# dmitrykoval/vinum

Measured on AMD Instinct MI355X. Metric: rows/sec + achieved HBM GB/s, filter->group-by over 10^9-row Arrow batches, higher is better.
Workload: dtype f64/int64; 1 GPU; configs[2]: SELECT k,sum(v),avg(v) WHERE v>63.9921875 GROUP BY k; N=1e+09 rows/GPU, G=1e+08 int64 keys, s=0.5; rows_per_gpu=1000000000, groups=100000000, group_count_hint=none: the operator samples the keys (what the reference boundary allows), parallelism=batch-sharded x1

## Files before the change

vinum_amd/csrc/vnm_agg.hip:

```cpp
#include <memory>
#include <algorithm>
#include <cmath>
#include <cstdlib>
#include <vector>

#include "vnm_agg.hpp"

namespace vnm {

constexpr uint64_t EMPTY = ~0ULL;
constexpr uint64_t LOCKED = ~0ULL - 1;
constexpr int AGG_BLOCK = 1024;
#ifndef VNM_AGG_R
#define VNM_AGG_R 8
#endif
constexpr int AGG_ROWS_PER_THREAD = VNM_AGG_R;
constexpr int AGG_TILE = AGG_BLOCK * AGG_ROWS_PER_THREAD;
constexpr int AGG_LDS_BUDGET = 128 * 1024;
constexpr int AGG_MAX_PROBES = 48;
constexpr int OG_BLOCK = 256;

struct GTable {
    uint64_t* tag;
    uint64_t* keyw;
// ... 197 lines not shown
            continue;
        }
        if (t == EMPTY) {
            uint64_t expected = EMPTY;
            if (__hip_atomic_compare_exchange_strong(&g.tag[h], &expected, LOCKED, __ATOMIC_RELAXED, __ATOMIC_RELAXED,
                                                     __HIP_MEMORY_SCOPE_AGENT)) {
                for (int i = 0; i < g.kwt; i++) st_agent(&g.keyw[(uint64_t)i * g.stride + h], kw[i]);
                asm volatile("s_waitcnt vmcnt(0)" ::: "memory");
                st_agent(&g.tag[h], tagv);
                atomicAdd(newc, 1u);
                return h;
            }
            continue;
        }
        if (t == LOCKED) continue;
        h = (h + 1) & mask;
    }
}

__device__ __forceinline__ void fold_new(const GTable& g, unsigned* s_new) {
    unsigned v = atomicExch(s_new, 0u);
    if (v) atomicAdd(&g.ctl[2], (unsigned long long)v);
}

__device__ __forceinline__ bool op_value(const AccOp& op, const vnm_dcol* cols, int64_t row, uint64_t* out) {
    if (op.kind == A_COUNT_ROWS) { *out = 1; return true; }
    const vnm_dcol& c = cols[op.col];
    if (!col_valid(c, row)) return false;
    switch (op.kind) {
        case A_COUNT_VALID: *out = 1; return true;
        case A_SUM_F64: *out = (uint64_t)__double_as_longlong(col_f64(c, row)); return true;
        case A_SUM_I64: *out = (uint64_t)col_i64(c, row); return true;
        case A_SUM_LO32: *out = (uint64_t)col_i64(c, row) & 0xFFFFFFFFULL; return true;
        case A_SUM_HI32S: *out = (uint64_t)(col_i64(c, row) >> 32); return true;
        case A_SUM_HI32U: *out = (uint64_t)col_i64(c, row) >> 32; return true;
        default:
            if (type_is_float(c.type)) *out = enc_f64(col_f64(c, row));
            else if (type_is_unsigned(c.type)) *out = (uint64_t)col_i64(c, row);
            else *out = enc_i64(col_i64(c, row));
            return true;
    }
}

__device__ __forceinline__ bool table_has_room(const AggArgs& a, unsigned* s_new) {
    fold_new(a.g, s_new);
    unsigned long long fill = __hip_atomic_load(&a.g.ctl[2], __ATOMIC_RELAXED, __HIP_MEMORY_SCOPE_AGENT);
    if ((int64_t)fill + a.margin > a.fill_limit) {
        __hip_atomic_store(&a.g.ctl[1], 1ULL, __ATOMIC_RELAXED, __HIP_MEMORY_SCOPE_AGENT);
        return false;
    }
    return true;
}

#include "vnm_agg_scan.inc"

#include "vnm_agg_tuple.inc"

#include "vnm_agg_onegroup.inc"

#include "vnm_agg_table.inc"

#include "vnm_agg_part.inc"

#include "vnm_agg_pack.inc"

#include "vnm_agg_dense.inc"

#include "vnm_agg_finalize.inc"

}

using namespace vnm;

struct DensePending {
    DFinalArgs df;
    int tb = 0, levels = 0, p1 = 0, fsplits = 1;
    int64_t nfinal = 0;
    int64_t dstride = 0;
    int64_t rows = 0;
    bool x_known = true;
    uint32_t x_inv = 0, x_exp = 0;
    bool exact_ok() const { return x_known && exact_adds_proved(((unsigned long long)x_exp << 32) | x_inv, rows); }
    std::vector<DSet> sets;
    std::vector<void*> blocks;
    DSet* dsets = nullptr;
    DTabSlot* table = nullptr;
    ~DensePending() { for (void* b : blocks) pool_free(b); pool_free(table); pool_free(dsets); }
};
constexpr size_t DP_MAX_SETS = 512;
struct DScanPending {
    DFinalArgs df{};
    DScanTable t{};
    int slots = 0;
    uint64_t* part_sum = nullptr;
    float* part_lo = nullptr;
    uint32_t* part_cnt = nullptr;
    unsigned long long* flags = nullptr;
    ~DScanPending() { pool_free(t.sum); pool_free(t.lo); pool_free(t.cnt); pool_free(part_sum); pool_free(part_lo); pool_free(part_cnt); pool_free(flags); }
};

struct vnm_agg {
    AggPlan plan;
    FuncOut outs[AGG_MAX_FUNCS];
    int n_funcs = 0;
    int func_col[AGG_MAX_FUNCS];
    int col_first_func[AGG_MAX_COLS];
    bool single = false;
    Predicate pred{};
    bool pred_set = false;
    int pred_op = 0, pred_is_float = 0;
    double pred_dval = 0;
    int64_t pred_ival = 0;
    int64_t hint = 0;
    GTable g{};
    bool have_table = false;
    int64_t rows_seen = 0;
    uint64_t* dkey = nullptr;
    uint64_t* dacc = nullptr;
    int64_t dstride = 0;
    int64_t n_groups = -1;
    std::vector<uint64_t> h_key, h_acc;
    bool host_ready = false;
    uint64_t* run_key = nullptr;
    uint64_t* run_acc = nullptr;
    int64_t run_stride = 0, run_n = 0;
    bool have_run = false;
    bool result_is_run = false;
    bool estimated = false;
    int64_t merge_stride = 0;
    unsigned long long* run_dir = nullptr;
    int64_t run_nfin = 0;
    vnm_agg* inner = nullptr;
    bool pack_tried = false;
    bool key_only_failed = false;
    int dense_state = 0;
    DenseMap dmap{};
    int64_t dense_span = 0;
    uint64_t dense_rlo = 0, dense_rhi = 0;
    bool rank_aligned = false;
    struct DensePending* pending = nullptr;
    double heavy_share = 0.0;
    int key_out_type = -1;
    std::vector<std::pair<int64_t, void*>> widened;
    bool widen_in[AGG_MAX_FUNCS] = {};
    bool any_widen_in = false;
    bool pred_lit_rounded = false;
    int pred_user_is_float = 0;
    double pred_user_dval = 0.0;
    int64_t pred_user_ival = 0;
    int fx_state = 0, fx_qe = 0;
    bool pack_null_seen = false;
    bool pring_off = false;
    bool fx_narrow = false;
    int fxn_state = 0, fxn_qe[3] = {0, 0, 0};
    bool null_inputs_seen = false;
    bool count8_off = false;
    int count_cb = 0;
    struct DScanPending* scan_pending = nullptr;
    bool dense_by_bound = false;
    bool range_given = false;
    int expr_col = -1;
    std::vector<vnm_expr_ins> expr_prog;
    int expr_ncols = 0;
    bool expr_fusable = false;
    bool expr_active = false;
    ExprProg expr_dev{};
    PackParams pack{};
    int c_funcs[AGG_MAX_FUNCS], c_in_types[AGG_MAX_FUNCS], c_in_flags[AGG_MAX_FUNCS], c_in_col_ids[AGG_MAX_FUNCS];
    bool c_has_ids = false;
    TDict tdict{};
    int64_t widest_est = 0;
    unsigned long long* tnext = nullptr;
    bool tuple_mode = false;
    std::vector<vnm_agg*> parts;
    std::vector<std::vector<int>> part_funcs;
    bool split_tried = false;
    bool async = false;
    struct QBatch { int64_t nrows; vnm_dcol key, col, pred; std::vector<vnm_dcol> ins; int64_t seq; };
    bool q_multi = false;
    std::vector<QBatch> q;
    int64_t q_rows = 0;
    bool q_pred_is_v = false;
    const std::vector<QBatch>* segs_active = nullptr;
    const uint8_t* kn_valid = nullptr;
    int64_t kn_off = 0;
    bool kn_failed = false;
    std::vector<VSeg> seg_host;
    struct vnm_agg_exact* ex = nullptr;
    bool child = false;
    int64_t seq = 0;
    int64_t cur_seq = -1;
};

namespace {

int table_alloc(vnm_agg* h, GTable* g, uint64_t cap, hipStream_t s) {
    memset(g, 0, sizeof(*g));
    g->cap = cap;
    g->stride = cap + 2;
    g->kwt = h->single || h->plan.n_keys == 0 ? 0 : h->plan.n_keys + 1;
    g->n_words = h->plan.n_words;
    g->tag = (uint64_t*)pool_alloc(g->stride * 8);
    g->acc = (uint64_t*)pool_alloc(g->stride * 8 * (size_t)g->n_words);
    g->ctl = (unsigned long long*)pool_alloc(64);
    if (g->kwt) g->keyw = (uint64_t*)pool_alloc(g->stride * 8 * (size_t)g->kwt);
    if (!g->tag || !g->acc || !g->ctl || (g->kwt && !g->keyw)) return 1;
    VNM_HIP(hipMemsetAsync(g->tag, 0xFF, g->stride * 8, s));
    VNM_HIP(hipMemsetAsync(g->ctl, 0, 64, s));
    for (int w = 0; w < g->n_words; w++) {
        const uint64_t init = merge_init(h->plan.merge[w]);
        if (init == 0 || init == ~0ULL) VNM_HIP(hipMemsetAsync(g->acc + (size_t)w * g->stride, init ? 0xFF : 0, g->stride * 8, s));
        else {
            fill_u64_kernel<<<(int)std::min<uint64_t>((g->stride + 255) / 256, (uint64_t)device_info().num_cus * 8), 256, 0, s>>>(g->acc + (size_t)w * g->stride, init, (int64_t)g->stride);
            VNM_HIP(hipGetLastError());
        }
    }
    return 0;
}

void table_free(GTable* g) {
    pool_free(g->tag);
    pool_free(g->acc);
    pool_free(g->keyw);
    pool_free(g->ctl);
    memset(g, 0, sizeof(*g));
}

uint64_t pow2_at_least(uint64_t x) {
    uint64_t p = 1;
    while (p < x) p <<= 1;
    return p;
}

int lds_slots_for(const AggPlan& p, int budget = AGG_LDS_BUDGET) {
    int per_slot = 8 * (1 + p.n_words);
    int s = 1;
    while ((s * 2 + 2) * per_slot <= budget) s *= 2;
    if (s > 8192) s = 8192;
    return s;
}

int table_grow(vnm_agg* h, uint64_t new_cap, hipStream_t s) {
    GTable old = h->g, ng;
    VNM_TRY(table_alloc(h, &ng, new_cap, s));
    MergeArgs m{};
    m.plan = h->plan;
    m.g = ng;
    m.n = (int64_t)old.stride;
    m.src_is_table = 1;
    m.src_stride = 1;
    m.src_tag = old.tag;
    m.src_cap = (int64_t)old.cap;
    for (int j = 0; j < old.kwt; j++) m.src_key[j] = old.keyw + (size_t)j * old.stride;
    for (int w = 0; w < old.n_words; w++) m.src_acc[w] = old.acc + (size_t)w * old.stride;
    int grid = device_info().num_cus * 8;
    agg_merge_kernel<<<grid, 256, 0, s>>>(m);
    VNM_HIP(hipGetLastError());
    VNM_HIP(hipStreamSynchronize(s));
    table_free(&old);
    h->g = ng;
    return 0;
}

int ensure_table(vnm_agg* h, int64_t nrows, hipStream_t s, bool rows_only = false) {
    if (h->have_table) return 0;
    uint64_t cap;
    if (h->plan.n_keys == 0) cap = 2;
    else {
        uint64_t want = h->hint > 0 ? (uint64_t)h->hint * 2 : (uint64_t)1 << 22;
        if ((h->hint <= 0 || rows_only) && (uint64_t)nrows * 2 < want) want = (uint64_t)(nrows > 512 ? nrows : 512) * 2;
        if (rows_only && want > (1ULL << 20)) want = 1ULL << 20;
        cap = pow2_at_least(want < 1024 ? 1024 : want);
    }
    VNM_TRY(table_alloc(h, &h->g, cap, s));
    h->have_table = true;
    return 0;
}

void invalidate_result(vnm_agg* h) {
    if (!h->result_is_run) {
        pool_free(h->dkey);
        pool_free(h->dacc);
    }
    h->result_is_run = false;
    h->dkey = h->dacc = nullptr;
    h->n_groups = -1;
    h->host_ready = false;
}

int64_t env_i64(const char* name, int64_t dflt) {
    const char* v = getenv(name);
    return v ? (int64_t)atoll(v) : dflt;
}

void drop_run(vnm_agg* h) {
    pool_free(h->run_key);
    pool_free(h->run_acc);
    pool_free(h->run_dir);
    h->run_dir = nullptr;
    h->run_nfin = 0;
    h->run_key = h->run_acc = nullptr;
    h->have_run = false;
    h->run_n = h->run_stride = 0;
}

int estimate_groups(vnm_agg* h, const vnm_dcol& key, int64_t nrows, int64_t* est, hipStream_t s, int64_t* tier0_lb = nullptr) {
// ... 866 lines not shown
```

vinum_amd/csrc/vnm_agg_dense.inc:

```

constexpr int DP_TBITS_MIN = 11, DP_TBITS_MAX = 13;
constexpr int DP_MAX_BITS = DP_TBITS_MAX + 18;

struct DenseMap {
    uint64_t lo_u;
    uint64_t sign;
    uint32_t mul;
    uint32_t mul_inv;
    uint32_t mask;
    int bits;
};

__device__ __forceinline__ uint64_t dense_key_of(const DenseMap& m, uint32_t codep) {
    const uint32_t code = (codep * m.mul_inv) & m.mask;
    return (m.lo_u + code) ^ m.sign;
}

struct DPartArgs {
    DenseMap map;
    const uint64_t* kp;
    const double* vp;
    const double* pp;
    int has_pred, pred_is_v, op;
    double thr;
    int64_t nrows;
    const VSeg* segs;
    int nseg;
    int64_t nsub;
    const double* vp2;
    const double* in_vals2;
    double* out_vals2;
    const uint8_t* kvalid;
    int64_t koff;
    uint64_t* nk_tag;
    uint64_t* nk_rows;
    uint64_t* nk_valid;
    uint64_t* nk_sum;
    int64_t nk_lo_stride;
    int has_expr;
    ExprProg expr;
    const double* in_vals;
    const uint32_t* in_codes;
    const uint32_t* in_counts;
    int64_t in_cap;
    int in_regions, in_split;
    int64_t in_pstride, in_rstride;
    int nt_store;
    int ready_list;
    int producer_major;
    int in_bits;
    double* out_vals;
    void* out_codes;
    uint32_t* out_counts;
    int64_t out_cap;
    int nparts;
    int out_bits;
    int in_pairs;
    unsigned long long* flags;
    ulonglong2* spill;
    int64_t spill_cap;
    const uint8_t* vvalid;
    int64_t voff;
    uint64_t* nspill;
    int64_t nspill_cap;
    double fx_q, fx_inv_q;
    int64_t fx_lim;
};
constexpr uint32_t DP_NULL32 = 0x80000000u;
__device__ __forceinline__ bool fx_encode(double v, double inv_q, int64_t* m, int64_t lim = 2147483647LL) {
    const double MAGIC = 6755399441055744.0;
    const double t = v * inv_q;
    const double u = t + MAGIC;
    const int64_t mm = (int64_t)(__double_as_longlong(u) - __double_as_longlong(MAGIC));
    *m = mm;
    return (u - MAGIC == t) && mm >= -lim && mm <= lim && __double_as_longlong(v) != (long long)0x8000000000000000ULL;
}
__device__ __forceinline__ double fx_bits(int64_t m) { return __longlong_as_double((long long)m); }
__device__ __forceinline__ int64_t fx_of(double carried) { return (int64_t)__double_as_longlong(carried); }
__device__ __forceinline__ void fx_expand(int64_t total, double q, double* hi, double* lo) {
    const double h = (double)total;
    const double l = (double)(total - (int64_t)h);
    *hi = h * q; *lo = l * q;
}

__device__ __forceinline__ void dense_spill(const DPartArgs& a, uint64_t key, double v, bool isnull = false) {
    if (isnull) {
        const unsigned long long pos = atomicAdd(&a.flags[3], 1ULL);
        if ((int64_t)pos < a.nspill_cap) a.nspill[pos] = key;
        else __hip_atomic_store(&a.flags[0], 1ULL, __ATOMIC_RELAXED, __HIP_MEMORY_SCOPE_AGENT);
        return;
    }
    const unsigned long long pos = atomicAdd(&a.flags[2], 1ULL);
    if ((int64_t)pos < a.spill_cap) a.spill[pos] = make_ulonglong2(key, (unsigned long long)__double_as_longlong(v));
    else __hip_atomic_store(&a.flags[0], 1ULL, __ATOMIC_RELAXED, __HIP_MEMORY_SCOPE_AGENT);
}
__device__ __forceinline__ void dense_spill_wave(const DPartArgs& a, bool want, uint64_t key, double v) {
    const unsigned long long m = __ballot(want);
    if (!m) return;
    const int lane = threadIdx.x & 63;
    const int leader = __ffsll((long long)m) - 1;
    unsigned long long base = 0;
    if (lane == leader) base = atomicAdd(&a.flags[2], (unsigned long long)__popcll(m));
    base = __shfl(base, leader);
    if (want) {
        const unsigned long long pos = base + (unsigned long long)__popcll(m & ((1ULL << lane) - 1ULL));
        if ((int64_t)pos < a.spill_cap) a.spill[pos] = make_ulonglong2(key, (unsigned long long)__double_as_longlong(v));
        else __hip_atomic_store(&a.flags[0], 1ULL, __ATOMIC_RELAXED, __HIP_MEMORY_SCOPE_AGENT);
    }
}
template <typename CT>
__device__ __forceinline__ CT dense_rem(uint32_t c, uint32_t remmask) {
    return (CT)((c & remmask) | ((c >> 31) << (sizeof(CT) * 8 - 1)));
}
template <typename CT>
__device__ __forceinline__ uint32_t dense_rem_code(CT r) { return (uint32_t)r & ((1u << (sizeof(CT) * 8 - 1)) - 1u); }
template <typename CT>
__device__ __forceinline__ bool dense_rem_null(CT r) { return ((uint32_t)r >> (sizeof(CT) * 8 - 1)) != 0; }

template <bool FROM_ROWS, typename CT, bool HAS_VAL = true, bool VN = false>
__global__ __launch_bounds__(PT_BLOCK) void dpart_scatter_kernel(DPartArgs a) {
    __shared__ double stage_v[HAS_VAL ? PT_TILE : 1];
    __shared__ uint32_t stage_c[PT_TILE];
    __shared__ uint32_t cnt[PT_MAXP], off[PT_MAXP], cursor[PT_MAXP];
    __shared__ uint32_t s_total;
    __shared__ uint32_t wtot[PT_MAXP / 64];
    const int tid = threadIdx.x;
    const int lane = tid & 63;
    const int np = a.nparts;
    const int npad = np < 64 ? 64 : np;
    const uint32_t remmask = (1u << a.out_bits) - 1u;
    for (int i = tid; i < PT_MAXP; i += PT_BLOCK) { cnt[i] = 0; cursor[i] = 0; }
    __syncthreads();

    int64_t out_base, out_stride;
    int64_t ntiles = 0;
    uint32_t prefix = 0;
    if (FROM_ROWS) {
        if (a.producer_major) { out_base = (int64_t)blockIdx.x * np; out_stride = 1; }
        else { out_base = blockIdx.x; out_stride = gridDim.x; }
        ntiles = (a.nrows + PT_TILE - 1) / PT_TILE;
    } else {
        const int pin = blockIdx.x / a.in_split, g = blockIdx.x % a.in_split;
        out_base = (int64_t)pin * np * a.in_split + g; out_stride = a.in_split;
        prefix = (uint32_t)pin << a.in_bits;
    }
    double* const ov = a.out_vals;
    CT* const oc = (CT*)a.out_codes;

    auto process_tile = [&](auto&& get_item, auto&& prefetch_next) {
        uint32_t myc[PT_ITEMS], myr[PT_ITEMS];
        double myv[PT_ITEMS];
#pragma unroll
        for (int k = 0; k < PT_ITEMS; k++) {
            myr[k] = 0xFFFFFFFFu;
            uint32_t c; double v;
            if (get_item(k, &c, &v)) {
                myc[k] = c;
                if (HAS_VAL) myv[k] = v;
                myr[k] = atomicAdd(&cnt[(c & ~DP_NULL32) >> a.out_bits], 1u);
            }
        }
        prefetch_next();
        __syncthreads();
        if (tid < npad) {
            uint32_t c = cnt[tid], inc = c;
#pragma unroll
            for (int d = 1; d < 64; d <<= 1) { uint32_t o = __shfl_up(inc, d); if (lane >= d) inc += o; }
            off[tid] = inc - c;
            if (lane == 63) wtot[tid >> 6] = inc;
        }
        __syncthreads();
        if (tid < npad) {
            uint32_t add = 0;
            for (int w = 0; w < (tid >> 6); w++) add += wtot[w];
            off[tid] += add;
            if (tid == npad - 1) s_total = off[tid] + cnt[tid];
        }
        __syncthreads();
#pragma unroll
        for (int k = 0; k < PT_ITEMS; k++) {
            if (myr[k] != 0xFFFFFFFFu) {
                const uint32_t pos = off[(myc[k] & ~DP_NULL32) >> a.out_bits] + myr[k];
                if (HAS_VAL) stage_v[pos] = myv[k];
                stage_c[pos] = myc[k];
            }
        }
        __syncthreads();
        const uint32_t total = s_total;
#pragma unroll
        for (int q = 0; q < PT_ITEMS; q++) {
            const uint32_t i = (uint32_t)q * PT_BLOCK + tid;
            bool lost = false;
            uint32_t c = 0;
            if (i < total) {
                c = stage_c[i];
                const uint32_t p = (c & ~DP_NULL32) >> a.out_bits;
                const uint32_t j = cursor[p] + (i - off[p]);
                if (j < (uint32_t)a.out_cap) {
                    const int64_t at = (out_base + (int64_t)p * out_stride) * a.out_cap + j;
                    if (a.nt_store) {
                        if (HAS_VAL) __builtin_nontemporal_store(stage_v[i], &ov[at]);
                        __builtin_nontemporal_store(dense_rem<CT>(c, remmask), &oc[at]);
                    } else {
                        if (HAS_VAL) ov[at] = stage_v[i];
                        oc[at] = dense_rem<CT>(c, remmask);
                    }
                } else lost = true;
            }
            if (lost && (c >> 31)) { dense_spill(a, dense_key_of(a.map, prefix | (c & ~DP_NULL32)), 0.0, true); lost = false; }
            dense_spill_wave(a, lost, dense_key_of(a.map, prefix | (c & ~DP_NULL32)), HAS_VAL && lost ? stage_v[i] : 0.0);
        }
        __syncthreads();
        if (tid < np) { cursor[tid] += cnt[tid]; cnt[tid] = 0; }
        __syncthreads();
    };

    if (FROM_ROWS) {
        ulonglong2 kk[PT_PAIRS];
        double2 vv[PT_PAIRS], pv[PT_PAIRS];
        uint8_t vb[VN ? PT_PAIRS : 1];
        auto load_rows = [&](int64_t tile) {
            const int64_t base = tile * PT_TILE;
            if (tile < ntiles && base + PT_TILE <= a.nrows) {
#pragma unroll
                for (int u = 0; u < PT_PAIRS; u++) {
                    const int64_t r = base + (int64_t)u * 2 * PT_BLOCK + 2 * tid;
                    kk[u] = *(const ulonglong2*)(a.kp + r);
                    if (HAS_VAL) vv[u] = a.has_expr ? expr_eval2(a.expr, r) : *(const double2*)(a.vp + r);
                    if (a.has_pred && !a.pred_is_v) pv[u] = *(const double2*)(a.pp + r);
                    if (VN) vb[VN ? u : 0] = (uint8_t)(a.vvalid[(a.voff + r) >> 3] >> ((a.voff + r) & 7));
                }
            }
        };
        load_rows(blockIdx.x);
        for (int64_t tile = blockIdx.x; tile < ntiles; tile += gridDim.x) {
            const int64_t base = tile * PT_TILE;
            const bool full = base + PT_TILE <= a.nrows;
            process_tile([&](int k, uint32_t* c, double* v) -> bool {
                const int u = k >> 1, el = k & 1;
                const int64_t r = base + (int64_t)u * 2 * PT_BLOCK + 2 * tid + el;
                if (r >= a.nrows) return false;
                uint64_t key; double val, p;
                bool isnull = false;
                if (full) {
                    key = el ? kk[u].y : kk[u].x;
                    val = HAS_VAL ? (el ? vv[u].y : vv[u].x) : 0.0;
                    p = a.pred_is_v ? val : (a.has_pred ? (el ? pv[u].y : pv[u].x) : 0.0);
                    if (VN) isnull = !((vb[VN ? u : 0] >> el) & 1);
                } else {
                    key = a.kp[r]; val = HAS_VAL ? (a.has_expr ? expr_eval1(a.expr, r) : a.vp[r]) : 0.0; p = a.has_pred ? (a.pred_is_v ? val : a.pp[r]) : 0.0;
                    if (VN) isnull = !((a.vvalid[(a.voff + r) >> 3] >> ((a.voff + r) & 7)) & 1);
                }
                if (VN && isnull && a.pred_is_v) return false;
                if (a.has_pred && !cmp_apply<double>(a.op, p, a.thr)) return false;
                const uint64_t d = (key ^ a.map.sign) - a.map.lo_u;
                if (d > (uint64_t)a.map.mask) { dense_spill(a, key, val, isnull); return false; }
                *c = (((uint32_t)d * a.map.mul) & a.map.mask) | (isnull ? DP_NULL32 : 0u);
                *v = isnull ? 0.0 : val;
                return true;
            }, [&]() { load_rows(tile + gridDim.x); });
        }
    } else {
        __shared__ uint32_t rstart[PT_MAX_REGIONS + 1];
        const int pin = blockIdx.x / a.in_split;
        const int per_max = (a.in_regions + a.in_split - 1) / a.in_split;
        const int g = blockIdx.x % a.in_split;
        const int first = g * per_max;
        const int per = first + per_max <= a.in_regions ? per_max : (a.in_regions > first ? a.in_regions - first : 0);
        const int64_t region0 = (int64_t)pin * a.in_pstride + (int64_t)first * a.in_rstride;
        if (tid == 0) {
            uint32_t run = 0;
            for (int rj = 0; rj < per; rj++) { rstart[rj] = run; run += (a.in_counts[region0 + rj * a.in_rstride] + 1) / 2; }
            rstart[per] = run;
        }
        __syncthreads();
        const uint32_t total_in = rstart[per];
        double2 ev[PT_PAIRS];
        uint2 ec[PT_PAIRS];
        uint32_t ok[PT_PAIRS];
        int reg[PT_PAIRS];
#pragma unroll
        for (int k = 0; k < PT_PAIRS; k++) reg[k] = 0;
        auto load_entries = [&](uint32_t t0) {
#pragma unroll
            for (int k = 0; k < PT_PAIRS; k++) {
                const uint32_t v = t0 + (uint32_t)k * PT_BLOCK + tid;
                ok[k] = 0;
                if (v < total_in) {
                    int lo = reg[k];
                    while (rstart[lo + 1] <= v) lo++;
                    reg[k] = lo;
                    const uint32_t e0 = 2u * (v - rstart[lo]);
                    const int64_t rg = region0 + lo * a.in_rstride;
                    const int64_t at = rg * a.in_cap + e0;
                    if (HAS_VAL) ev[k] = *(const double2*)(a.in_vals + at);
                    ec[k] = *(const uint2*)(a.in_codes + at);
                    ok[k] = e0 + 1 < a.in_counts[rg] ? 3u : 1u;
                }
            }
        };
        load_entries(0);
        for (uint32_t t0 = 0; t0 < total_in; t0 += PT_TILE / 2) {
            process_tile([&](int k, uint32_t* c, double* v) -> bool {
                const int u = k >> 1, el = k & 1;
                if (!((ok[u] >> el) & 1u)) return false;
                *c = el ? ec[u].y : ec[u].x;
                *v = HAS_VAL ? (el ? ev[u].y : ev[u].x) : 0.0;
                return true;
            }, [&]() { load_entries(t0 + PT_TILE / 2); });
        }
    }
    if (tid < np) a.out_counts[out_base + (int64_t)tid * out_stride] = cursor[tid] < (uint32_t)a.out_cap ? cursor[tid] : (uint32_t)a.out_cap;
}

__device__ __forceinline__ void exact_track(double v, uint32_t& xinv, uint32_t& xexp) {
    const uint64_t b = (uint64_t)__double_as_longlong(v) & 0x7FFFFFFFFFFFFFFFULL;
    if (b == 0) return;
    const uint32_t hi = (uint32_t)(b >> 32), lo = (uint32_t)b;
    const uint32_t e = hi >> 20;
    const uint32_t mh = (hi & 0xFFFFFu) | (e ? 0x100000u : 0u);
    const uint32_t tz = lo ? (uint32_t)__builtin_ctz(lo) : 32u + (uint32_t)__builtin_ctz(mh);
    const uint32_t low = (e ? e : 1u) + tz;
    xinv = max(xinv, 0xFFFFu - low);
    xexp = max(xexp, e);
}
static inline bool exact_adds_proved(unsigned long long word, int64_t rows) {
    const uint32_t xinv = (uint32_t)word, xexp = (uint32_t)(word >> 32);
    if (xinv == 0 && xexp == 0) return true;
    if (xexp >= 2047) return false;
    int lg = 0;
    while (((int64_t)1 << lg) < rows) lg++;
    return (int64_t)lg + (int64_t)xexp <= (int64_t)(0xFFFFu - xinv);
}

constexpr int DR_FB = 16;
typedef double dr_v2 __attribute__((ext_vector_type(2)));
typedef uint32_t dr_u2 __attribute__((ext_vector_type(2)));
template <bool FROM_ROWS, typename CT, bool HAS_VAL, int DR_BLOCK, int DR_PAIRS, bool PV = false, bool VN = false, int MAXR = 0, bool SEG = false, bool KN = false,
          bool V2 = false, bool FX = false, bool W32 = false>
__global__ __launch_bounds__(DR_BLOCK) void dring_scatter_kernel(DPartArgs a, int ring_cap) {
    extern __shared__ uint64_t dr_lds[];
    static_assert(!FX || (HAS_VAL && !V2), "fixed-point entries: one value (VN: only where the filter drops the NULL rows, vn_fold)");
    static_assert(!W32 || FX, "32-bit entry words are fixed-point words");
    constexpr int FB = W32 ? 32 : DR_FB, EPL = FB / 8;
    constexpr int NE = 2 * DR_PAIRS;
    const int np = a.nparts;
    double* const rv = (double*)dr_lds;
    double* const rv2 = rv + (V2 ? (size_t)np * ring_cap : 0);
    CT* const rc = (CT*)(dr_lds + (HAS_VAL ? (size_t)np * ring_cap * (V2 ? 2 : 1) : 0));
    __shared__ uint32_t fill[PT_MAXP], head[PT_MAXP], cursor[PT_MAXP];
    __shared__ uint32_t s_retry[2];
    __shared__ uint32_t s_nready[2];
    __shared__ uint16_t ready[2][PT_MAXP];
    __shared__ uint32_t s_spill[3];
    const int tid = threadIdx.x;
    const uint32_t remmask = (1u << a.out_bits) - 1u;
    for (int i = tid; i < PT_MAXP; i += DR_BLOCK) { fill[i] = 0; head[i] = 0; cursor[i] = 0; }
    if (tid < 2) { s_retry[tid] = 0; s_nready[tid] = 0; }
    int ph = 0;
    const bool use_list = a.ready_list != 0;
    if (tid == 0) s_spill[0] = 0;
    __syncthreads();

    int64_t out_base, out_stride;
    uint32_t prefix = 0;
    if (FROM_ROWS) {
        if (a.producer_major) { out_base = (int64_t)blockIdx.x * np; out_stride = 1; }
        else { out_base = blockIdx.x; out_stride = gridDim.x; }
    } else {
        const int pin = blockIdx.x / a.in_split, g = blockIdx.x % a.in_split;
        out_base = (int64_t)pin * np * a.in_split + g; out_stride = a.in_split;
        prefix = (uint32_t)pin << a.in_bits;
    }
    double* const ov = a.out_vals;
    double* const ov2 = a.out_vals2;
    CT* const oc = (CT*)a.out_codes;
    const uint32_t ocap = (uint32_t)a.out_cap;

    auto insert = [&](uint32_t c, double v, double w2) -> bool {
        const uint32_t p = (c & ~DP_NULL32) >> a.out_bits;
        const uint32_t r = atomicAdd(&fill[p], 1u);
        if (r == (uint32_t)FB - 1u && use_list) ready[ph][atomicAdd(&s_nready[ph], 1u)] = (uint16_t)p;
        if (r >= (uint32_t)ring_cap) return false;
        uint32_t slot = head[p] + r;
        if (slot >= (uint32_t)ring_cap) slot -= ring_cap;
        if (W32) {
            ((uint32_t*)rv)[(size_t)p * ring_cap + slot] = ((uint32_t)(int32_t)fx_of(v) << a.out_bits) | (c & remmask);
            return true;
        }
        if (FX) {
            ((uint64_t*)rv)[(size_t)p * ring_cap + slot] = ((uint64_t)fx_of(v) << a.out_bits) | (uint64_t)(c & remmask);
            return true;
        }
        if (HAS_VAL) rv[(size_t)p * ring_cap + slot] = v;
        if (V2) rv2[(size_t)p * ring_cap + slot] = w2;
        rc[(size_t)p * ring_cap + slot] = dense_rem<CT>(c, remmask);
        return true;
    };
    auto fx_rem = [&](size_t li) -> uint32_t { return W32 ? ((const uint32_t*)rv)[li] & remmask : (uint32_t)(((const uint64_t*)rv)[li] & (uint64_t)remmask); };
    auto fx_val = [&](size_t li) -> double {
        return W32 ? (double)((int32_t)((const uint32_t*)rv)[li] >> a.out_bits) * a.fx_q : (double)((int64_t)((const uint64_t*)rv)[li] >> a.out_bits) * a.fx_q;
    };
    auto flush = [&](bool drain) {
        const int j = tid & 7;
        const bool listed = use_list && !drain;
        const int nwalk = listed ? (int)s_nready[ph] : np;
        for (int q = tid >> 3; q < nwalk; q += DR_BLOCK / 8) {
            const int p = listed ? (int)ready[ph][q] : q;
            uint32_t f = fill[p];
            if (f > (uint32_t)ring_cap) f = ring_cap;
            const uint32_t nb = drain ? (f + FB - 1) / FB : f / FB;
            if (nb == 0) continue;
            const uint32_t h = head[p], cur = cursor[p];
            const int64_t rbase = (out_base + (int64_t)p * out_stride) * a.out_cap;
            uint32_t done = 0, wrote = 0;
            for (uint32_t b = 0; b < nb; b++) {
                uint32_t src = h + b * FB;
                if (src >= (uint32_t)ring_cap) src -= ring_cap;
                const uint32_t n_here = f - b * FB < (uint32_t)FB ? f - b * FB : FB;
                const size_t li = (size_t)p * ring_cap + src + EPL * j;
                if (cur + wrote + FB <= ocap) {
                    const int64_t at = rbase + cur + wrote + EPL * j;
                    if ((uint32_t)(EPL * j) < n_here) {
                        if (W32) {
                            const dr_v2 x = *(const dr_v2*)((const uint32_t*)rv + li);
                            if (a.nt_store) __builtin_nontemporal_store(x, (dr_v2*)((uint32_t*)ov + at)); else *(dr_v2*)((uint32_t*)ov + at) = x;
                        } else if (HAS_VAL) {
                            const dr_v2 x = *(const dr_v2*)(rv + li);
                            if (a.nt_store) __builtin_nontemporal_store(x, (dr_v2*)(ov + at)); else *(dr_v2*)(ov + at) = x;
                        }
                        if (V2) {
                            const dr_v2 x2 = *(const dr_v2*)(rv2 + li);
                            if (a.nt_store) __builtin_nontemporal_store(x2, (dr_v2*)(ov2 + at)); else *(dr_v2*)(ov2 + at) = x2;
                        }
                        if (FX) {
                        } else if (sizeof(CT) == 4) {
                            const dr_u2 y = *(const dr_u2*)(rc + li);
                            if (a.nt_store) __builtin_nontemporal_store(y, (dr_u2*)(oc + at)); else *(dr_u2*)(oc + at) = y;
                        } else {
                            const uint32_t y = *(const uint32_t*)(rc + li);
                            if (a.nt_store) __builtin_nontemporal_store(y, (uint32_t*)(oc + at)); else *(uint32_t*)(oc + at) = y;
                        }
                    }
                    wrote += n_here;
                } else if (V2) {
                    if (j == 0) __hip_atomic_store(&a.flags[0], 1ULL, __ATOMIC_RELAXED, __HIP_MEMORY_SCOPE_AGENT);
                } else if (!drain && a.nspill == nullptr) {
                    const unsigned long long m = __ballot(j == 0);
                    const int lane = tid & 63;
                    const int leader = __ffsll((long long)m) - 1;
                    unsigned long long base = 0;
                    if (lane == leader) base = atomicAdd(&a.flags[2], (unsigned long long)__popcll(m) * FB);
                    base = __shfl(base, leader);
                    const unsigned long long pos = base + (unsigned long long)__popcll(m & ((1ULL << (lane - j)) - 1ULL)) * FB + EPL * j;
                    if ((int64_t)(pos + EPL) <= a.spill_cap) {
                        for (int e = 0; e < EPL; e++)
                            a.spill[pos + e] = make_ulonglong2(dense_key_of(a.map, prefix | (p << a.out_bits) | (FX ? fx_rem(li + e) : dense_rem_code<CT>(rc[FX ? 0 : li + e]))),
                                                               (unsigned long long)__double_as_longlong(FX ? fx_val(li + e) : (HAS_VAL ? rv[li + e] : 0.0)));
                    } else __hip_atomic_store(&a.flags[0], 1ULL, __ATOMIC_RELAXED, __HIP_MEMORY_SCOPE_AGENT);
                } else {
                    for (int e = 0; e < EPL; e++)
                        if ((uint32_t)(EPL * j + e) < n_here) {
                            if (FX) dense_spill(a, dense_key_of(a.map, prefix | (p << a.out_bits) | fx_rem(li + e)), fx_val(li + e));
                            else dense_spill(a, dense_key_of(a.map, prefix | (p << a.out_bits) | dense_rem_code<CT>(rc[FX ? 0 : li + e])), HAS_VAL ? rv[li + e] : 0.0,
                                             dense_rem_null<CT>(rc[FX ? 0 : li + e]));
                        }
                }
                done += n_here;
            }
            if (j == 0) {
                uint32_t nh = h + nb * FB;
                while (nh >= (uint32_t)ring_cap) nh -= ring_cap;
                head[p] = drain ? 0 : nh;
                fill[p] = f - done;
                cursor[p] = cur + wrote;
            }
        }
    };
    int maxr = MAXR;
    auto rounds = [&](const uint32_t (&c)[NE], const double (&v)[NE], const double (&w2)[V2 ? NE : 1], uint32_t okmask) {
        uint32_t pend = 0;
        int nr = 0;
#pragma unroll
        for (int e = 0; e < NE; e++) if (((okmask >> e) & 1u) && !insert(c[e], v[e], w2[V2 ? e : 0])) pend |= 1u << e;
        for (;;) {
            if (pend) s_retry[ph] = 1;
            __syncthreads();
            flush(false);
            if (tid == 0) { s_retry[ph ^ 1] = 0; s_nready[ph ^ 1] = 0; }
            __syncthreads();
            const bool again = s_retry[ph] != 0;
            ph ^= 1;
            if (!again) break;
            if (MAXR > 0 && ++nr >= maxr) {
                uint32_t mine = 0;
#pragma unroll
                for (int e = 0; e < NE; e++) {
                    if (((pend >> e) & 1u) && (c[e] >> 31)) {
                        dense_spill(a, dense_key_of(a.map, prefix | (c[e] & ~DP_NULL32)), 0.0, true);
                        pend &= ~(1u << e);
                    }
                }
                mine = (uint32_t)__popc(pend);
                uint32_t at = mine ? atomicAdd(&s_spill[0], mine) : 0u;
                __syncthreads();
                if (tid == 0) {
                    const unsigned long long base = atomicAdd(&a.flags[2], (unsigned long long)s_spill[0]);
                    s_spill[1] = (uint32_t)base; s_spill[2] = (uint32_t)(base >> 32);
                }
                __syncthreads();
                const unsigned long long base = ((unsigned long long)s_spill[2] << 32) | s_spill[1];
#pragma unroll
                for (int e = 0; e < NE; e++) {
                    if ((pend >> e) & 1u) {
                        const unsigned long long pos = base + at++;
                        if ((int64_t)pos < a.spill_cap)
                            a.spill[pos] = make_ulonglong2(dense_key_of(a.map, prefix | c[e]),
                                                           (unsigned long long)__double_as_longlong(FX ? (double)fx_of(v[e]) * a.fx_q : (HAS_VAL ? v[e] : 0.0)));
                        else __hip_atomic_store(&a.flags[0], 1ULL, __ATOMIC_RELAXED, __HIP_MEMORY_SCOPE_AGENT);
                    }
                }
                __syncthreads();
                if (tid == 0) s_spill[0] = 0;
                maxr = MAXR - 1;
                break;
            }
#pragma unroll
            for (int e = 0; e < NE; e++) if (((pend >> e) & 1u) && insert(c[e], v[e], w2[V2 ? e : 0])) pend &= ~(1u << e);
        }
    };

    double nk_hi = -0.0, nk_lo = 0.0;
    uint32_t nk_cnt = 0;
    constexpr bool XT = FROM_ROWS && HAS_VAL && !V2 && !FX;
    uint32_t xinv = 0, xexp = 0;
    bool fx_bad = false;
    if (FROM_ROWS && !SEG) {
        const int64_t sub = (int64_t)NE * DR_BLOCK;
        const int64_t nsub = (a.nrows + sub - 1) / sub;
        const int64_t nfull = a.nrows / sub;
        ulonglong2 kk[DR_PAIRS];
        double2 vv[DR_PAIRS], pv[PV ? DR_PAIRS : 1], vv2[V2 ? DR_PAIRS : 1];
        uint32_t vbits = 0;
        uint32_t kbits = 0;
        auto load_sub = [&](int64_t st) {
            if (st < nfull) {
                if (VN) vbits = 0;
                if (KN) kbits = 0;
#pragma unroll
                for (int u = 0; u < DR_PAIRS; u++) {
                    const int64_t r = st * sub + (int64_t)u * 2 * DR_BLOCK + 2 * tid;
                    kk[u] = *(const ulonglong2*)(a.kp + r);
                    if (HAS_VAL) vv[u] = *(const double2*)(a.vp + r);
                    if (V2) vv2[V2 ? u : 0] = *(const double2*)(a.vp2 + r);
                    if (PV) pv[u] = *(const double2*)(a.pp + r);
                    if (VN) vbits |= (((uint32_t)a.vvalid[(a.voff + r) >> 3] >> ((a.voff + r) & 7)) & 3u) << (2 * u);
                    if (KN) kbits |= (((uint32_t)a.kvalid[(a.koff + r) >> 3] >> ((a.koff + r) & 7)) & 3u) << (2 * u);
                }
            }
        };
        load_sub(blockIdx.x);
        for (int64_t st = blockIdx.x; st < nsub; st += gridDim.x) {
            uint32_t c[NE]; double v[NE]; double w2[V2 ? NE : 1]; uint32_t okmask = 0;
#pragma unroll
            for (int e = 0; e < NE; e++) {
                const int u = e >> 1, el = e & 1;
                const int64_t r = st * sub + (int64_t)u * 2 * DR_BLOCK + 2 * tid + el;
                c[e] = 0; v[e] = 0.0;
                if (r >= a.nrows) continue;
                uint64_t key; double val, p, val2 = 0.0;
                bool isnull = false, keynull = false;
                if (st < nfull) {
                    if (KN) keynull = !((kbits >> e) & 1u);
                    key = el ? kk[u].y : kk[u].x;
                    val = HAS_VAL ? (el ? vv[u].y : vv[u].x) : 0.0;
                    if (V2) val2 = el ? vv2[V2 ? u : 0].y : vv2[V2 ? u : 0].x;
                    p = PV ? (el ? pv[PV ? u : 0].y : pv[PV ? u : 0].x) : val;
                    if (VN) isnull = !((vbits >> e) & 1u);
                } else {
                    key = a.kp[r]; val = HAS_VAL ? a.vp[r] : 0.0; p = a.has_pred ? (a.pred_is_v ? val : a.pp[r]) : 0.0;
                    if (V2) val2 = a.vp2[r];
                    if (VN) isnull = !((a.vvalid[(a.voff + r) >> 3] >> ((a.voff + r) & 7)) & 1);
                    if (KN) keynull = !((a.kvalid[(a.koff + r) >> 3] >> ((a.koff + r) & 7)) & 1);
                }
                if (VN && isnull && a.pred_is_v) continue;
                if (a.has_pred && !cmp_apply<double>(a.op, p, a.thr)) continue;
                if (KN && keynull) {
                    nk_cnt++;
                    const double t = nk_hi + val;
                    nk_lo += two_sum_err(nk_hi, val, t);
                    nk_hi = t;
                    continue;
                }
                const uint64_t d = (key ^ a.map.sign) - a.map.lo_u;
                if (d > (uint64_t)a.map.mask) {
                    if (V2) __hip_atomic_store(&a.flags[0], 1ULL, __ATOMIC_RELAXED, __HIP_MEMORY_SCOPE_AGENT);
                    else dense_spill(a, key, val, isnull);
                    continue;
                }
                c[e] = (((uint32_t)d * a.map.mul) & a.map.mask) | (VN && isnull ? DP_NULL32 : 0u);
                v[e] = VN && isnull ? 0.0 : val;
                if (FX) { int64_t m; if (!fx_encode(val, a.fx_inv_q, &m, a.fx_lim)) { fx_bad = true; continue; } v[e] = fx_bits(m); }
                if (V2) w2[V2 ? e : 0] = val2;
                if (XT) exact_track(v[e], xinv, xexp);
                okmask |= 1u << e;
            }
            load_sub(st + gridDim.x);
            rounds(c, v, w2, okmask);
        }
    } else if (FROM_ROWS) {
        const int64_t sub = (int64_t)NE * DR_BLOCK;
        struct Cur { const uint64_t* kp; const double* vp; const double* pp; const uint8_t* vvalid; int64_t voff; int64_t nrows; int64_t lst; };
        const int nseg = a.nseg;
        const VSegConst segs = seg_table(a.segs);
        const int64_t nsub = a.nsub;
        int sg = 0;
        auto locate = [&](int64_t st, Cur& c) {
            while (sg + 1 < nseg && st >= segs[sg + 1].first_tile) sg++;
            c.kp = segs[sg].kp; c.vp = (const double*)segs[sg].vp; c.pp = segs[sg].pp;
            c.vvalid = VN ? segs[sg].vvalid : nullptr; c.voff = VN ? segs[sg].voff : 0;
            c.nrows = segs[sg].nrows;
            c.lst = st - segs[sg].first_tile;
        };
        ulonglong2 kk[DR_PAIRS];
        double2 vv[DR_PAIRS], pv[PV ? DR_PAIRS : 1];
        uint32_t vbits = 0;
        auto load_sub = [&](const Cur& c) {
            if (c.lst < c.nrows / sub) {
                if (VN) vbits = 0;
#pragma unroll
                for (int u = 0; u < DR_PAIRS; u++) {
                    const int64_t r = c.lst * sub + (int64_t)u * 2 * DR_BLOCK + 2 * tid;
                    kk[u] = *(const ulonglong2*)(c.kp + r);
                    if (HAS_VAL) vv[u] = *(const double2*)(c.vp + r);
                    if (PV) pv[u] = *(const double2*)(c.pp + r);
                    if (VN) vbits |= (((uint32_t)c.vvalid[(c.voff + r) >> 3] >> ((c.voff + r) & 7)) & 3u) << (2 * u);
                }
            }
        };
        Cur cur{}, nxt{};
        if ((int64_t)blockIdx.x < nsub) { locate(blockIdx.x, cur); load_sub(cur); }
        for (int64_t st = blockIdx.x; st < nsub; st += gridDim.x) {
            uint32_t c[NE]; double v[NE]; uint32_t okmask = 0;
            const bool full = cur.lst < cur.nrows / sub;
#pragma unroll
            for (int e = 0; e < NE; e++) {
                const int u = e >> 1, el = e & 1;
                const int64_t r = cur.lst * sub + (int64_t)u * 2 * DR_BLOCK + 2 * tid + el;
                c[e] = 0; v[e] = 0.0;
                if (r >= cur.nrows) continue;
                uint64_t key; double val, p;
                bool isnull = false;
                if (full) {
                    key = el ? kk[u].y : kk[u].x;
                    val = HAS_VAL ? (el ? vv[u].y : vv[u].x) : 0.0;
                    p = PV ? (el ? pv[PV ? u : 0].y : pv[PV ? u : 0].x) : val;
                    if (VN) isnull = !((vbits >> e) & 1u);
                } else {
                    key = cur.kp[r]; val = HAS_VAL ? cur.vp[r] : 0.0; p = a.has_pred ? (a.pred_is_v ? val : cur.pp[r]) : 0.0;
                    if (VN) isnull = !((cur.vvalid[(cur.voff + r) >> 3] >> ((cur.voff + r) & 7)) & 1);
                }
                if (VN && isnull && a.pred_is_v) continue;
                if (a.has_pred && !cmp_apply<double>(a.op, p, a.thr)) continue;
                const uint64_t d = (key ^ a.map.sign) - a.map.lo_u;
                if (d > (uint64_t)a.map.mask) { dense_spill(a, key, val, isnull); continue; }
                c[e] = (((uint32_t)d * a.map.mul) & a.map.mask) | (VN && isnull ? DP_NULL32 : 0u);
                v[e] = VN && isnull ? 0.0 : val;
                if (FX) { int64_t m; if (!fx_encode(val, a.fx_inv_q, &m, a.fx_lim)) { fx_bad = true; continue; } v[e] = fx_bits(m); }
                if (XT) exact_track(v[e], xinv, xexp);
                okmask |= 1u << e;
            }
            if (st + gridDim.x < nsub) { locate(st + gridDim.x, nxt); load_sub(nxt); }
            const double w2[V2 ? NE : 1] = {};
            rounds(c, v, w2, okmask);
            cur = nxt;
        }
    } else {
        __shared__ uint32_t rstart[PT_MAX_REGIONS + 1];
        const int pin = blockIdx.x / a.in_split;
        const int per_max = (a.in_regions + a.in_split - 1) / a.in_split;
        const int g = blockIdx.x % a.in_split;
        const int first = g * per_max;
        const int per = first + per_max <= a.in_regions ? per_max : (a.in_regions > first ? a.in_regions - first : 0);
        const int64_t region0 = (int64_t)pin * a.in_pstride + (int64_t)first * a.in_rstride;
        if (tid == 0) {
            uint32_t run = 0;
            for (int rj = 0; rj < per; rj++) { rstart[rj] = run; run += (a.in_counts[region0 + rj * a.in_rstride] + 1) / 2; }
            rstart[per] = run;
        }
        __syncthreads();
        const uint32_t total_in = rstart[per];
        double2 ev[DR_PAIRS], ev2[V2 ? DR_PAIRS : 1];
        uint2 ec[DR_PAIRS];
        uint32_t okm = 0;
        int reg = 0;
        auto load_pairs = [&](uint32_t t0) {
            okm = 0;
#pragma unroll
            for (int u = 0; u < DR_PAIRS; u++) {
                const uint32_t v = t0 + (uint32_t)u * DR_BLOCK + tid;
                if (v < total_in) {
                    int lo = reg;
                    while (rstart[lo + 1] <= v) lo++;
                    reg = lo;
                    const uint32_t e0 = 2u * (v - rstart[lo]);
                    const int64_t rg = region0 + lo * a.in_rstride;
                    const int64_t at = rg * a.in_cap + e0;
                    if (HAS_VAL) ev[u] = *(const double2*)(a.in_vals + at);
                    if (V2) ev2[V2 ? u : 0] = *(const double2*)(a.in_vals2 + at);
                    if (!FX) ec[u] = *(const uint2*)(a.in_codes + at);
                    okm |= (e0 + 1 < a.in_counts[rg] ? 3u : 1u) << (2 * u);
                }
            }
        };
        load_pairs(0);
        for (uint32_t t0 = 0; t0 < total_in; t0 += DR_PAIRS * DR_BLOCK) {
            uint32_t c[NE]; double v[NE]; double w2[V2 ? NE : 1];
#pragma unroll
            for (int u = 0; u < DR_PAIRS; u++) {
                if (FX) {
                    const uint64_t w0 = (uint64_t)__double_as_longlong(ev[u].x), w1 = (uint64_t)__double_as_longlong(ev[u].y);
                    const uint64_t inmask = ((uint64_t)1 << a.in_bits) - 1;
                    c[2 * u] = (uint32_t)(w0 & inmask); c[2 * u + 1] = (uint32_t)(w1 & inmask);
                    v[2 * u] = fx_bits((int64_t)w0 >> a.in_bits); v[2 * u + 1] = fx_bits((int64_t)w1 >> a.in_bits);
                    continue;
                }
                c[2 * u] = ec[u].x; c[2 * u + 1] = ec[u].y;
                v[2 * u] = HAS_VAL ? ev[u].x : 0.0; v[2 * u + 1] = HAS_VAL ? ev[u].y : 0.0;
                if (V2) { w2[V2 ? 2 * u : 0] = ev2[V2 ? u : 0].x; w2[V2 ? 2 * u + 1 : 0] = ev2[V2 ? u : 0].y; }
            }
            const uint32_t okmask = okm;
            load_pairs(t0 + DR_PAIRS * DR_BLOCK);
            rounds(c, v, w2, okmask);
        }
    }
    flush(true);
    __syncthreads();
    if (tid < np) a.out_counts[out_base + (int64_t)tid * out_stride] = cursor[tid];
    if (FX && FROM_ROWS) { if (__syncthreads_or(fx_bad ? 1 : 0) && tid == 0) __hip_atomic_store(&a.flags[7], 1ULL, __ATOMIC_RELAXED, __HIP_MEMORY_SCOPE_AGENT); }
    if (XT) {
        if (tid < 2) s_spill[tid] = 0;
        __syncthreads();
        if (xinv) atomicMax(&s_spill[0], xinv);
        if (xexp) atomicMax(&s_spill[1], xexp);
        __syncthreads();
        if (tid < 2 && s_spill[tid]) atomicMax((uint32_t*)&a.flags[6] + tid, s_spill[tid]);
    }
    if (KN) {
        __shared__ uint64_t s_nk[3];
        __syncthreads();
        if (tid < 3) s_nk[tid] = tid == 0 ? F64_NEG_ZERO : 0;
        __syncthreads();
        if (nk_cnt) {
            l_add_f64c(&s_nk[0], 1, nk_hi);
            __hip_atomic_fetch_add((double*)&s_nk[1], nk_lo, __ATOMIC_RELAXED, __HIP_MEMORY_SCOPE_WORKGROUP);
            __hip_atomic_fetch_add(&s_nk[2], (uint64_t)nk_cnt, __ATOMIC_RELAXED, __HIP_MEMORY_SCOPE_WORKGROUP);
        }
        __syncthreads();
        if (tid == 0 && s_nk[2]) {
            if (ld_agent(a.nk_tag) == EMPTY) st_agent(a.nk_tag, 0);
            if (a.nk_rows) __hip_atomic_fetch_add(a.nk_rows, s_nk[2], __ATOMIC_RELAXED, __HIP_MEMORY_SCOPE_AGENT);
            if (a.nk_valid) __hip_atomic_fetch_add(a.nk_valid, s_nk[2], __ATOMIC_RELAXED, __HIP_MEMORY_SCOPE_AGENT);
            if (a.nk_sum) {
                if (a.nk_lo_stride) {
                    g_add_f64c(a.nk_sum, a.nk_lo_stride, __longlong_as_double((long long)s_nk[0]));
                    __hip_atomic_fetch_add((double*)(a.nk_sum + a.nk_lo_stride), __longlong_as_double((long long)s_nk[1]), __ATOMIC_RELAXED, __HIP_MEMORY_SCOPE_AGENT);
                } else __hip_atomic_fetch_add((double*)a.nk_sum, __longlong_as_double((long long)s_nk[0]) + __longlong_as_double((long long)s_nk[1]), __ATOMIC_RELAXED, __HIP_MEMORY_SCOPE_AGENT);
            }
        }
    }
}

__global__ void dnull_fold_kernel(const unsigned long long* scr, uint64_t* tag, uint64_t* rows, uint64_t* valid, uint64_t* sum, int64_t lo_stride) {
    if (threadIdx.x != 0 || blockIdx.x != 0) return;
    if (!(scr[1] | scr[2])) return;
    if (ld_agent(tag) == EMPTY) st_agent(tag, 0);
    if (rows) __hip_atomic_fetch_add(rows, scr[1], __ATOMIC_RELAXED, __HIP_MEMORY_SCOPE_AGENT);
    if (valid) __hip_atomic_fetch_add(valid, scr[2], __ATOMIC_RELAXED, __HIP_MEMORY_SCOPE_AGENT);
    if (sum) {
        if (lo_stride) {
            g_add_f64c(sum, lo_stride, __longlong_as_double((long long)scr[3]));
            __hip_atomic_fetch_add((double*)(sum + lo_stride), __longlong_as_double((long long)scr[4]), __ATOMIC_RELAXED, __HIP_MEMORY_SCOPE_AGENT);
        } else __hip_atomic_fetch_add((double*)sum, __longlong_as_double((long long)scr[3]), __ATOMIC_RELAXED, __HIP_MEMORY_SCOPE_AGENT);
    }
}

struct DSet {
    const double* vals; const void* codes; const uint32_t* counts;
    int64_t cap, pstride, rstride;
    int regions, pad;
};
__device__ __forceinline__ const double* dfin_words(const double* base, int64_t entries, bool w32) {
    return w32 ? (const double*)((const uint32_t*)base + entries) : base + entries;
}
constexpr int DF_MAX_OUT = 8;
enum { DF_RUN = 0, DF_COLS = 1, DF_TABLE = 2 };
enum { DF_KEY = 0, DF_SUM = 1, DF_AVG = 2, DF_COUNT = 3 };
struct DTabSlot { double sum; float lo; uint32_t cnt; };
struct DFinalArgs {
    int64_t pstride, rstride;
    DenseMap map;
    const double* vals;
    const void* codes;
    const uint32_t* counts;
    int64_t cap;
    int regions;
    int64_t nfinal;
    int w_rows, w_valid, w_sum, w_lo;
    uint64_t* dkey;
    uint64_t* dacc;
    int64_t dstride;
    unsigned long long* flags;
    int splits;
    uint64_t* part_sum;
    float* part_lo;
    uint32_t* part_cnt;
    int n_out;
    int out_kind[DF_MAX_OUT];
    int key_width;
    void* out_ptr[DF_MAX_OUT];
    DTabSlot* table;
    const DSet* sets;
    int nsets;
    int sub_bits, sub;
    int has_side;
    GTable side;
    const uint32_t* side_bloom;
    uint32_t side_bloom_mask;
    uint8_t* side_found;
    int64_t* null_pos;
    const double* vals2;
    int w_valid2, w_sum2, w_lo2;
    double fx_q;
    int fx_w32;
    int pack_n;
    int key_field[DF_MAX_OUT];
    int pack_shift[AGG_MAX_KEYS], pack_bits[AGG_MAX_KEYS];
    uint64_t pack_lo[AGG_MAX_KEYS];
};
__device__ __forceinline__ uint64_t df_key_cell(const DFinalArgs& a, int c, uint64_t key) {
    if (!a.pack_n) return key;
    const int f = a.key_field[c];
    return ((key >> a.pack_shift[f]) & ((1ULL << a.pack_bits[f]) - 1ULL)) + a.pack_lo[f];
}
__device__ __forceinline__ void df_store_cell(const DFinalArgs& a, int c, int64_t pos, uint64_t cell) {
    if (a.out_kind[c] == DF_KEY && a.key_width && a.key_width != 8) {
        if (a.key_width == 4) ((uint32_t*)a.out_ptr[c])[pos] = (uint32_t)cell;
        else if (a.key_width == 2) ((uint16_t*)a.out_ptr[c])[pos] = (uint16_t)cell;
        else ((uint8_t*)a.out_ptr[c])[pos] = (uint8_t)cell;
        return;
    }
    ((uint64_t*)a.out_ptr[c])[pos] = cell;
}
constexpr int DSIDE_BLOOM_BITS = 1 << 16;
__device__ __forceinline__ uint32_t dside_bloom_bit(uint64_t k, uint32_t mask) { return hash_u64(k ^ 0xD6E8FEB86659FD93ULL) & mask; }
__device__ __forceinline__ uint32_t dside_bloom_pattern(uint64_t k, uint32_t b) {
    const uint32_t h2 = hash_u64(k * 0x9E3779B97F4A7C15ULL + 0x632BE59BD9B4E019ULL);
    return (1u << (b & 31)) | (1u << ((h2 >> 7) & 31));
}
__device__ __forceinline__ void dside_merge(const DFinalArgs& a, const uint32_t* lb, uint64_t key, double& hi, double& lo, uint64_t& cnt) {
    const GTable& g = a.side;
    uint64_t slot = ~0ULL;
    if (key == EMPTY) { if (g.tag[g.cap] != EMPTY) slot = g.cap; }
    else {
        const uint32_t bb = dside_bloom_bit(key, a.side_bloom_mask);
        const uint32_t word = (lb && a.side_bloom_mask == DSIDE_BLOOM_BITS - 1) ? lb[bb >> 5] : a.side_bloom[bb >> 5];
        const uint32_t pat = dside_bloom_pattern(key, bb);
        if ((word & pat) != pat) return;
        const uint64_t mask = g.cap - 1;
        uint64_t h = hash_u64(key) & mask;
        for (uint64_t probes = 0; probes <= mask; probes++) {
            const uint64_t t = g.tag[h];
            if (t == key) { slot = h; break; }
            if (t == EMPTY) break;
            h = (h + 1) & mask;
        }
    }
    if (slot == ~0ULL) return;
    const int wc = a.w_rows >= 0 ? a.w_rows : a.w_valid;
    if (wc >= 0) cnt += g.acc[(uint64_t)wc * g.stride + slot];
    if (a.w_sum >= 0) {
        const double sh = __longlong_as_double((long long)g.acc[(uint64_t)a.w_sum * g.stride + slot]);
        const double t = hi + sh;
        lo += two_sum_err(hi, sh, t);
        if (a.w_lo >= 0) lo += __longlong_as_double((long long)g.acc[(uint64_t)a.w_lo * g.stride + slot]);
        hi = t;
    }
    a.side_found[slot] = 1;
}
__global__ __launch_bounds__(256) void dside_bloom_kernel(GTable g, uint32_t* bloom, uint32_t bmask) {
    const int64_t stride = (int64_t)gridDim.x * 256;
    for (int64_t slot = (int64_t)blockIdx.x * 256 + threadIdx.x; slot < (int64_t)g.cap; slot += stride) {
// ... 1083 lines not shown
            for (uint32_t i0 = 0; i0 < n; i0 += 64 * 4 * 2) {
                uint4 q[2];
#pragma unroll
                for (int u = 0; u < 2; u++) {
                    const uint32_t i = i0 + ((uint32_t)u * 64 + lane) * 4;
                    if (i < n) q[u] = *(const uint4*)(sc + i);
                }
#pragma unroll
                for (int u = 0; u < 2; u++) {
                    const uint32_t i = i0 + ((uint32_t)u * 64 + lane) * 4;
                    const uint32_t c4[4] = {q[u].x, q[u].y, q[u].z, q[u].w};
#pragma unroll
                    for (int k = 0; k < 4; k++) {
                        if (i + k >= n) continue;
                        const uint32_t code = c4[k];
                        if ((code >> tb8) != sub) continue;
                        const uint32_t b = code & ((1u << tb8) - 1u), sh = (b & (uint32_t)(PER - 1)) * (uint32_t)CB;
                        const uint32_t old = atomicAdd(&dc_tab[b >> PSH], 1u << sh);
                        over |= ((old >> sh) & CMASK) == CMASK;
                    }
                }
            }
        }
        if (over) s_over = 1;
        __syncthreads();
        if (s_over) {
            if (tid == 0) { __hip_atomic_store(&a.flags[5], 1ULL, __ATOMIC_RELAXED, __HIP_MEMORY_SCOPE_AGENT); __hip_atomic_store(&a.flags[0], 1ULL, __ATOMIC_RELAXED, __HIP_MEMORY_SCOPE_AGENT); }
            return;
        }
        uint32_t mine = 0;
        for (int i = tid; i < (1 << (tb8 - PSH)); i += 1024) {
            const uint32_t x = dc_tab[i];
            if (CB == 8) mine += ((x & 0xffu) != 0) + ((x & 0xff00u) != 0) + ((x & 0xff0000u) != 0) + ((x >> 24) != 0);
            else mine += ((x & 0xffffu) != 0) + ((x >> 16) != 0);
        }
        pa_block_add(&s_n, mine);
        __syncthreads();
        const uint32_t ngroups = s_n;
        __syncthreads();
        if (tid == 0) { s_base = atomicAdd(&a.flags[1], (unsigned long long)ngroups); s_n = 0; }
        __syncthreads();
        if ((int64_t)(s_base + ngroups) > a.dstride) {
            if (tid == 0) __hip_atomic_store(&a.flags[0], 1ULL, __ATOMIC_RELAXED, __HIP_MEMORY_SCOPE_AGENT);
            return;
        }
        const uint32_t prefix = ((uint32_t)p << (tb8 + sub_bits)) | (sub << tb8);
        for (int i0 = 0; i0 < (1 << tb8); i0 += 1024) {
            const int i = i0 + tid;
            const uint32_t cnt = (dc_tab[i >> PSH] >> ((i & (PER - 1)) * CB)) & CMASK;
            const bool occ = cnt != 0;
            const uint64_t b = __ballot(occ);
            uint32_t wbase = 0;
            if (lane == 0 && b) wbase = atomicAdd(&s_n, (uint32_t)__popcll(b));
            wbase = __shfl(wbase, 0);
            if (occ) {
                const uint64_t lt = lane == 0 ? 0ULL : (~0ULL >> (64 - lane));
                dgen_write_group(a, (int64_t)s_base + wbase + __popcll(b & lt), prefix | (uint32_t)i, cnt, nullptr);
            }
        }
        __syncthreads();
    }
}

struct DScanTable {
    double* sum;
    double* lo;
    unsigned long long* cnt;
};
__global__ __launch_bounds__(512) void dscan_accumulate_kernel(const uint64_t* part_sum, const float* part_lo, const uint32_t* part_cnt,
                                                                int splits, int slots, DScanTable t) {
    __shared__ double s_hi[8][64], s_lo[8][64];
    __shared__ unsigned long long s_cnt[8][64];
    const int li = threadIdx.x & 63, g = threadIdx.x >> 6;
    const int i = blockIdx.x * 64 + li;
    double hi = -0.0, lo = 0.0;
    unsigned long long cnt = 0;
    constexpr int U = 4;
    for (int sp0 = g; sp0 < splits; sp0 += 8 * U) {
        uint32_t c[U]; uint64_t xs[U]; float xl[U];
#pragma unroll
        for (int u = 0; u < U; u++) {
            const int sp = sp0 + 8 * u;
            c[u] = 0; xs[u] = 0; xl[u] = 0.0f;
            if (sp < splits && i < slots) {
                const size_t at = (size_t)sp * slots + i;
                c[u] = part_cnt[at]; xs[u] = part_sum[at]; xl[u] = part_lo[at];
            }
        }
#pragma unroll
        for (int u = 0; u < U; u++) {
            if (c[u] == 0) continue;
            cnt += c[u];
            const double x = __longlong_as_double((long long)xs[u]);
            const double s = hi + x;
            lo += two_sum_err(hi, x, s) + (double)xl[u];
            hi = s;
        }
    }
    s_hi[g][li] = hi; s_lo[g][li] = lo; s_cnt[g][li] = cnt;
    __syncthreads();
    if (g != 0 || i >= slots) return;
    for (int gg = 1; gg < 8; gg++) {
        const unsigned long long c = s_cnt[gg][li];
        if (c == 0) continue;
        cnt += c;
        const double x = s_hi[gg][li];
        const double s = hi + x;
        lo += two_sum_err(hi, x, s) + s_lo[gg][li];
        hi = s;
    }
    if (cnt == 0) return;
    const double old = t.sum[i], s = old + hi;
    t.lo[i] += two_sum_err(old, hi, s) + lo;
    t.sum[i] = s;
    t.cnt[i] += cnt;
}
__global__ __launch_bounds__(512) void dscan_emit_kernel(DFinalArgs a, int slots, DScanTable t) {
    __shared__ uint32_t s_n;
    __shared__ unsigned long long s_base;
    const int tid = threadIdx.x, lane = tid & 63;
    const int i = blockIdx.x * 512 + tid;
    if (tid == 0) s_n = 0;
    __syncthreads();
    const unsigned long long cnt = i < slots ? t.cnt[i] : 0ULL;
    const bool occ = cnt != 0;
    pa_block_add(&s_n, occ ? 1u : 0u);
    __syncthreads();
    const uint32_t ngroups = s_n;
    __syncthreads();
    if (tid == 0) { s_base = atomicAdd(&a.flags[1], (unsigned long long)ngroups); s_n = 0; }
    __syncthreads();
    if ((int64_t)(s_base + ngroups) > a.dstride) {
        if (tid == 0) __hip_atomic_store(&a.flags[0], 1ULL, __ATOMIC_RELAXED, __HIP_MEMORY_SCOPE_AGENT);
        return;
    }
    const uint64_t b = __ballot(occ);
    uint32_t wbase = 0;
    if (lane == 0 && b) wbase = atomicAdd(&s_n, (uint32_t)__popcll(b));
    wbase = __shfl(wbase, 0);
    if (occ) {
        const uint64_t lt = lane == 0 ? 0ULL : (~0ULL >> (64 - lane));
        const int64_t pos = (int64_t)s_base + wbase + __popcll(b & lt);
        const double hi = t.sum[i], lo = t.lo[i];
        a.dkey[pos] = dense_key_of(a.map, (uint32_t)i);
        a.dkey[a.dstride + pos] = 0;
        if (a.w_rows >= 0) a.dacc[(int64_t)a.w_rows * a.dstride + pos] = cnt;
        if (a.w_valid >= 0) a.dacc[(int64_t)a.w_valid * a.dstride + pos] = cnt;
        if (a.w_sum >= 0) a.dacc[(int64_t)a.w_sum * a.dstride + pos] = (uint64_t)__double_as_longlong(hi);
        if (a.w_lo >= 0) a.dacc[(int64_t)a.w_lo * a.dstride + pos] = (uint64_t)__double_as_longlong(lo);
        else if (a.w_sum >= 0) a.dacc[(int64_t)a.w_sum * a.dstride + pos] = (uint64_t)__double_as_longlong(fsum2(hi, lo));
    }
}

__global__ __launch_bounds__(256) void fx_sample_kernel(const double* vals, int64_t nrows, int64_t m, unsigned long long* out) {
    __shared__ uint32_t sx[2];
    if (threadIdx.x < 2) sx[threadIdx.x] = 0;
    __syncthreads();
    const int64_t stride = (int64_t)gridDim.x * blockDim.x;
    uint32_t xinv = 0, xexp = 0;
    for (int64_t i = (int64_t)blockIdx.x * blockDim.x + threadIdx.x; i < m; i += stride) exact_track(vals[(int64_t)(((__int128)i * nrows) / m)], xinv, xexp);
    if (xinv) atomicMax(&sx[0], xinv);
    if (xexp) atomicMax(&sx[1], xexp);
    __syncthreads();
    if (threadIdx.x < 2 && sx[threadIdx.x]) atomicMax((uint32_t*)out + threadIdx.x, sx[threadIdx.x]);
}

__global__ __launch_bounds__(256) void dense_sample_range_kernel(const uint64_t* keys, int64_t nrows, int64_t m, uint64_t sign,
                                                                 unsigned long long* out, const uint8_t* kvalid, int64_t koff) {
    __shared__ unsigned long long smn[4], smx[4];
    const int64_t stride = (int64_t)gridDim.x * blockDim.x;
    uint64_t mn = ~0ULL, mx = 0;
    for (int64_t i = (int64_t)blockIdx.x * blockDim.x + threadIdx.x; i < m; i += stride) {
        const int64_t row = (int64_t)(((__int128)i * nrows) / m);
        if (!key_row_valid(kvalid, koff, row)) continue;
        const uint64_t ku = keys[row] ^ sign;
        mn = ku < mn ? ku : mn;
        mx = ku > mx ? ku : mx;
    }
#pragma unroll
    for (int o = 32; o > 0; o >>= 1) {
        const uint64_t omn = __shfl_xor(mn, o), omx = __shfl_xor(mx, o);
        mn = omn < mn ? omn : mn;
        mx = omx > mx ? omx : mx;
    }
    if ((threadIdx.x & 63) == 0) { smn[threadIdx.x >> 6] = mn; smx[threadIdx.x >> 6] = mx; }
    __syncthreads();
    if (threadIdx.x == 0) {
        for (int w = 1; w < 4; w++) { mn = smn[w] < mn ? smn[w] : mn; mx = smx[w] > mx ? smx[w] : mx; }
        atomicMin(&out[0], (unsigned long long)mn);
        atomicMax(&out[1], (unsigned long long)mx);
    }
}
```

vinum_amd/csrc/vnm_agg_routes.inc:

```
namespace {
template <class F>
int pick_bool(bool b, F&& f) { return b ? f(std::true_type{}) : f(std::false_type{}); }
template <int LO, int HI, class F>
int pick_int(int v, F&& f) {
    if constexpr (LO < HI) { if (v > LO) return pick_int<LO + 1, HI>(v, f); }
    return f(std::integral_constant<int, LO>{});
}
template <class F>
int pick_out(int out, F&& f) {
    if (out == DF_COLS) return f(std::integral_constant<int, DF_COLS>{});
    if (out == DF_TABLE) return f(std::integral_constant<int, DF_TABLE>{});
    return f(std::integral_constant<int, DF_RUN>{});
}
template <class K, class Q, class... A>
int launch_resident_as(K kernel, Q occ_kernel, int64_t work, int block, size_t lds, int occ_max, hipStream_t s, const A&... args) {
    if (lds) VNM_HIP(hipFuncSetAttribute((const void*)kernel, hipFuncAttributeMaxDynamicSharedMemorySize, (int)lds));
    int occ = 0;
    if (hipOccupancyMaxActiveBlocksPerMultiprocessor(&occ, (const void*)occ_kernel, block, lds) != hipSuccess || occ < 1) occ = 1;
    const int grid = (int)std::min<int64_t>(work, (int64_t)device_info().num_cus * std::min(occ, occ_max));
    kernel<<<grid, block, lds, s>>>(args...);
    return 0;
}
template <class K, class... A>
int launch_resident(K kernel, int64_t work, int block, size_t lds, int occ_max, hipStream_t s, const A&... args) {
    return launch_resident_as(kernel, kernel, work, block, lds, occ_max, s, args...);
}
template <class K, class... A>
int launch_dyn(K kernel, int grid, int block, size_t lds, hipStream_t s, const A&... args) {
    VNM_HIP(hipFuncSetAttribute((const void*)kernel, hipFuncAttributeMaxDynamicSharedMemorySize, (int)lds));
    kernel<<<grid, block, lds, s>>>(args...);
    return 0;
}
template <class K>
int launch_part_final(K kernel, int64_t work, size_t lds, hipStream_t s, const PartAggArgs& pa) {
    const int cus = device_info().num_cus;
    if (lds) VNM_HIP(hipFuncSetAttribute((const void*)kernel, hipFuncAttributeMaxDynamicSharedMemorySize, (int)lds));
    int grid = (int)std::min<int64_t>(work, (int64_t)cus * 4), occ = 0;
    if (hipOccupancyMaxActiveBlocksPerMultiprocessor(&occ, (const void*)kernel, PA_BLOCK, lds) == hipSuccess && occ > 0)
        grid = (int)std::min<int64_t>(work, (int64_t)cus * std::min(occ, (int)env_i64("VNM_PA_OCC", 8)));
    kernel<<<grid, PA_BLOCK, lds, s>>>(pa);
    return 0;
}

struct RingLaunch { int grid, cap, pairs; bool limit, seg, kn; hipStream_t s; };
constexpr int ring_flush_block(bool w32) { return w32 ? 32 : DR_FB; }
inline bool ring_one_round(int pairs, int nparts, int cap, bool w32) { return 2 * pairs * 1024 <= nparts * (cap - ring_flush_block(w32)); }
inline int ring_sub_tile_pairs(int want, bool pv, bool limit, int nparts, int cap, bool w32) {
    int pr = want >= 4 && !pv ? 4 : (want >= 2 ? 2 : 1);
    while (limit && pr > 1 && !ring_one_round(pr, nparts, cap, w32)) pr >>= 1;
    return pr;
}
inline int ring_cap_for(int np, size_t esize) {
    int cap = (int)((size_t)(env_i64("VNM_DENSE_RING_LDS", 128) * 1024) / ((size_t)np * esize) / DR_FB) * DR_FB;
    cap = std::min(cap, (int)env_i64("VNM_DENSE_RING_CAP", std::max(80, ((8192 / np + DR_FB + DR_FB - 1) / DR_FB) * DR_FB)));
    if (np < env_i64("VNM_DENSE_RING_MIN_NP", 32)) return 0;
    return cap >= 2 * DR_FB ? cap : 0;
}
inline int ring_cap_w32(int np) {
    const int cap = std::min(256, (int)((size_t)128 * 1024 / ((size_t)np * 4) / 32) * 32);
    return cap >= 64 ? cap : 0;
}

template <bool FR, typename CT, bool HV, int PR, bool PV, bool VN, int MAXR, bool SEG, bool KN, bool V2, bool FX, bool W32>
int launch_ring(int grid, const DPartArgs& d, int cap, hipStream_t s) {
    constexpr size_t esize = FX ? (W32 ? 4 : 8) : (HV ? (V2 ? 16 : 8) : 0) + sizeof(CT);
    const size_t lds = (((size_t)d.nparts * cap * esize) + 15) & ~(size_t)15;
    return launch_dyn(dring_scatter_kernel<FR, CT, HV, 1024, PR, PV, VN, MAXR, SEG, KN, V2, FX, W32>, grid, 1024, lds, s, d, cap);
}
template <bool FR, typename CT, bool HV, bool PV, bool VN, bool FX, bool W32, int PR>
int ring_scatter_pairs(const RingLaunch& r, const DPartArgs& d) {
    auto go = [&](auto lim, auto seg, auto kn) {
        return launch_ring<FR, CT, HV, PR, PV, VN, decltype(lim)::value ? 2 : 0, decltype(seg)::value, decltype(kn)::value, false, FX, W32>(r.grid, d, r.cap, r.s);
    };
    return pick_bool(r.limit && ring_one_round(PR, d.nparts, r.cap, W32), [&](auto lim) {
        if constexpr (FR && HV && !VN) {
            if (r.kn) return go(lim, std::false_type{}, std::true_type{});
            if (r.seg) return go(lim, std::true_type{}, std::false_type{});
        }
        return go(lim, std::false_type{}, std::false_type{});
    });
}
template <bool FR, typename CT, bool HV, bool PV, bool VN, bool FX = false, bool W32 = false>
int ring_scatter(const RingLaunch& r, const DPartArgs& d) {
    if constexpr (!PV) {
        if (r.pairs == 4) return ring_scatter_pairs<FR, CT, HV, PV, VN, FX, W32, 4>(r, d);
    }
    if (r.pairs >= 2) return ring_scatter_pairs<FR, CT, HV, PV, VN, FX, W32, 2>(r, d);
    return ring_scatter_pairs<FR, CT, HV, PV, VN, FX, W32, 1>(r, d);
}


int partitioned_aggregate(vnm_agg* h, const AggArgs& a, int64_t nrows, hipStream_t s, ulonglong2** spill_out = nullptr,
                          int64_t* n_spill_out = nullptr) {
    const int cus = device_info().num_cus;
    const int64_t l1_cap = env_i64("VNM_AGG_PART_L1_MAX", 256) * 512;
    const bool small_tables = a.part_generic && (size_t)(PA_SLOTS + 1) * 8 * (1 + h->plan.n_words) > 54 * 1024 &&
                              h->hint / 450 < l1_cap && getenv("VNM_AGG_NO_SMALL_TABLES") == nullptr;
    int pa_slots = small_tables ? PA_SLOTS / 2 : PA_SLOTS;
    while (a.part_generic && pa_slots > 256 && (size_t)(pa_slots + 1) * 8 * (1 + h->plan.n_words) > 150 * 1024) pa_slots /= 2;
    const int64_t per_final = env_i64("VNM_AGG_PART_GROUPS", 900 * pa_slots / PA_SLOTS);
    int64_t nfin = 2;
    while (nfin * per_final < h->hint) nfin *= 2;
    const int64_t l1_max = env_i64("VNM_AGG_PART_L1_MAX", 256);
    if (nfin > l1_max * 512) {
        if (h->hint / (l1_max * 512) > 1600 * pa_slots / PA_SLOTS) return 2;
        nfin = l1_max * 512;
    }
    const int E = a.part_wide ? 1 + h->plan.n_cols + (a.part_vmask ? 1 : 0) : 2;
    const bool wide = a.part_wide != 0;
    const int64_t tile1 = wide ? pw_tile(E) : PT_TILE;
    const size_t ebytes = (size_t)E * 8;
    const int levels = nfin > std::min<int64_t>(l1_max * 2, PT_MAXP) ? 2 : 1;
    const int np1 = levels == 2 ? (int)l1_max : (int)nfin;
    const int np2 = levels == 2 ? (int)(nfin / l1_max) : 0;
    const int grid1 = (int)std::min<int64_t>((int64_t)cus * 2, (nrows + tile1 - 1) / tile1);
    const int split2 = std::max(2, (grid1 + PT_MAX_REGIONS - 1) / PT_MAX_REGIONS);
    const int64_t tiles_per_wg = ((nrows + tile1 - 1) / tile1 + grid1 - 1) / grid1;
    const int64_t rows_per_wg = tiles_per_wg * tile1;
    const double slack = std::max(0.0, 4.5 / std::sqrt((double)std::max<int64_t>(per_final, 16) / 2.0));
    const int64_t cap1 = rows_per_wg / np1 + (int64_t)((double)(rows_per_wg / np1) * std::max(0.2, slack)) + 512;
    PoolScope pool;
    unsigned long long* flags = (unsigned long long*)pool.take(64);
    ulonglong2* e1 = (ulonglong2*)pool.take((size_t)np1 * grid1 * cap1 * ebytes);
    uint32_t* c1 = (uint32_t*)pool.take((size_t)np1 * grid1 * 4);
    if (!flags || !e1 || !c1) return 1;
    VNM_HIP(hipMemsetAsync(flags, 0, 64, s));
    const int64_t spill_cap = spill_out ? nrows / 2 + (1 << 20) : 0;
    ulonglong2* spill = spill_out ? (ulonglong2*)pool.take((size_t)spill_cap * (wide ? ebytes : 16)) : nullptr;
    if (spill_out && !spill) return 1;
    PartArgs p1{};
    p1.kp = (const uint64_t*)a.keys[0].values + a.keys[0].offset;
    p1.vp = h->plan.n_cols ? (const double*)a.cols[0].values + a.cols[0].offset : (const double*)p1.kp;
    p1.has_expr = a.has_expr; p1.expr = a.expr;
    p1.pp = h->pred_set ? (const double*)a.pred.values + a.pred.offset : nullptr;
    p1.has_pred = h->pred_set; p1.pred_is_v = a.hot_pred_is_v; p1.op = a.p.op; p1.thr = a.p.dval;
    p1.nrows = nrows;
    p1.out_entries = e1; p1.out_counts = c1; p1.out_cap = cap1;
    int lg1 = 0;
    while ((1 << lg1) < np1) lg1++;
    p1.nparts = np1; p1.shift = 32 - lg1; p1.flags = flags;
    p1.debug = (int)env_i64("VNM_PART_DEBUG", 0);
    p1.spill = spill; p1.spill_cap = spill_cap;
    p1.nval = h->plan.n_cols;
    p1.has_vmask = a.part_vmask;
    if (wide) {
        for (int c = 0; c < h->plan.n_cols; c++) p1.vcols[c] = a.cols[c];
        p1.wp = a.p;
        p1.wpred = a.pred;
    }
    auto pring_cap = [&](int np) -> int { int cap = (int)((size_t)128 * 1024 / 16 / (size_t)np); cap = std::min(cap, 64) / 16 * 16; return cap; };
    auto pring_lds = [&](int np) -> size_t { return (size_t)np * pring_cap(np) * 16; };
    const bool ring_ok = !wide && !a.has_expr && !h->pring_off && env_i64("VNM_PART_RING", 7) != 0 && (a.keys[0].offset & 1) == 0 && (!h->plan.n_cols || (a.cols[0].offset & 1) == 0) &&
                         (!h->pred_set || a.hot_pred_is_v || (a.pred.offset & 1) == 0) && h->plan.n_cols > 0;
    const bool ring1 = ring_ok && np1 <= 256 && np1 >= 128 && (env_i64("VNM_PART_RING", 7) & 1);
    const bool ring2 = ring_ok && levels == 2 && np2 <= 256 && np2 >= 128 && (env_i64("VNM_PART_RING", 7) & 2);
    const bool ring2_512 = ring_ok && levels == 2 && np2 == 512 && (env_i64("VNM_PART_RING", 7) & 4);
    {
        KernelTimer timer("agg_part_scatter1", s);
        if (ring1) VNM_TRY(pick_bool(p1.has_pred && !p1.pred_is_v, [&](auto pv) { return launch_dyn(pring_scatter_kernel<true, 2, 16, decltype(pv)::value>, grid1, PT_BLOCK, pring_lds(np1), s, p1, pring_cap(np1)); }));
        else if (!wide) part_scatter_kernel<true><<<grid1, PT_BLOCK, 0, s>>>(p1);
        else VNM_TRY((pick_int<1, 7>(E, [&](auto e) { return launch_dyn(part_scatter_wide_kernel<true, decltype(e)::value, pw_items(decltype(e)::value)>, grid1, PT_BLOCK, (size_t)pw_tile(E) * ebytes, s, p1); })));
    }
    VNM_HIP(hipGetLastError());
    auto overflowed = [&]() -> int {
        unsigned long long f = 0;
        if (hipMemcpyAsync(&f, flags, 8, hipMemcpyDeviceToHost, s) != hipSuccess || hipStreamSynchronize(s) != hipSuccess) return -1;
        return f ? 1 : 0;
    };
    {
        int ov = overflowed();
        if (ov > 0 && ring1) {
            h->pring_off = true;
            route_note("hash_partitions:rings_failed", "a region overflowed or a sub-tile needed too many rounds: the tile-sorting scatter takes the batch and every later one");
            pool.done(e1); pool.done(c1); pool.done(flags); pool.done(spill);
            return partitioned_aggregate(h, a, nrows, s, spill_out, n_spill_out);
        }
        if (ov) return ov < 0 ? set_error("aggregate: partition pass failed") : 2;
    }
    if (ring1) route_note("hash_partitions:rings", "%d x %d partitions: (key, value) entries through LDS rings, whole 256-byte blocks out", np1, np2);

    const ulonglong2* fin_e = e1;
    const uint32_t* fin_c = c1;
    int64_t fin_cap = cap1, nfinal = np1;
    int fin_regions = grid1;
    ulonglong2* e2 = nullptr;
    uint32_t* c2 = nullptr;
    if (levels == 2) {
        const int64_t per_pg = (int64_t)grid1 * rows_per_wg / np1 / split2;
        const int64_t cap2 = per_pg / np2 + (int64_t)((double)(per_pg / np2) * std::max(0.25, slack)) + 256;
        e2 = (ulonglong2*)pool.take((size_t)np1 * np2 * split2 * cap2 * ebytes);
        c2 = (uint32_t*)pool.take((size_t)np1 * np2 * split2 * 4);
        if (!e2 || !c2) return 1;
        PartArgs p2{};
        p2.in_entries = e1; p2.in_counts = c1; p2.in_cap = cap1; p2.in_regions = grid1; p2.in_split = split2;
        p2.out_entries = e2; p2.out_counts = c2; p2.out_cap = cap2;
        p2.nparts = np2; p2.shift = 15; p2.flags = flags;
        p2.debug = p1.debug;
        p2.spill = spill; p2.spill_cap = spill_cap;
        p2.nval = h->plan.n_cols;
        p2.has_vmask = a.part_vmask;
        {
            KernelTimer timer("agg_part_scatter2", s);
            const int g2 = np1 * p2.in_split;
            if (ring2) VNM_TRY(launch_dyn(pring_scatter_kernel<false, 2, 16, false>, g2, PT_BLOCK, pring_lds(np2), s, p2, pring_cap(np2)));
            else if (ring2_512) VNM_TRY(launch_dyn(pring_scatter_kernel<false, 1, 8, false>, g2, PT_BLOCK, (size_t)512 * 16 * 16, s, p2, 16));
            else if (!wide) part_scatter_kernel<false><<<g2, PT_BLOCK, 0, s>>>(p2);
            else VNM_TRY((pick_int<1, 7>(E, [&](auto e) {
                constexpr int EW = decltype(e)::value;
                if constexpr (EW <= 2) { if (np2 < 128) return launch_dyn(part_scatter_wide_kernel<false, EW, 4>, g2, PT_BLOCK, (size_t)PT_BLOCK * 4 * ebytes, s, p2); }
                return launch_dyn(part_scatter_wide_kernel<false, EW, pw_items(EW)>, g2, PT_BLOCK, (size_t)PT_BLOCK * pw_items(EW) * ebytes, s, p2);
            })));
        }
        VNM_HIP(hipGetLastError());
        {
            int ov = overflowed();
            if (ov > 0 && (ring2 || ring2_512)) {
                h->pring_off = true;
                route_note("hash_partitions:rings_failed", "level 2: a region overflowed or a sub-tile needed too many rounds: the tile-sorting scatter takes the batch and every later one");
                pool.done(e1); pool.done(c1); pool.done(e2); pool.done(c2); pool.done(flags); pool.done(spill);
                return partitioned_aggregate(h, a, nrows, s, spill_out, n_spill_out);
            }
            if (ov) return ov < 0 ? set_error("aggregate: partition pass failed") : 2;
        }
        fin_e = e2; fin_c = c2; fin_cap = cap2; nfinal = (int64_t)np1 * np2; fin_regions = p2.in_split;
    }

    int splits = 1;
    if (nfinal < (int64_t)cus * 4) {
        splits = (int)std::min<int64_t>(256, ((int64_t)cus * 8 + nfinal - 1) / nfinal);
        if (splits > fin_regions) splits = fin_regions;
    }
    const bool to_table = splits > 1 && !(h->have_table || h->have_run);
    const bool dup_run = splits > 1 && !to_table;
    const int64_t dstride = to_table ? 2 : std::min<int64_t>(nrows, (h->hint * 2 + (1 << 20)) * (dup_run ? splits : 1)) + 2;
    uint64_t* rk = (uint64_t*)pool.take((size_t)dstride * 8 * 2);
    uint64_t* ra = (uint64_t*)pool.take((size_t)dstride * 8 * h->plan.n_words);
    if (!rk || !ra) return 1;
    unsigned long long* dir = nullptr;
    if (!to_table && !dup_run) {
        dir = (unsigned long long*)pool.take((size_t)nfinal * 16);
        if (!dir) return 1;
// ... 331 lines not shown
        break;
    }
    return set_error("aggregate: no dense final pass of form %d for tables of 2^%d slots (internal error)", form, TB);
}
int launch_dense_final(const DFinalArgs& df, int tb, int out, bool lo64, hipStream_t s, bool exact = false, const DSet* only_set = nullptr) {
    KernelTimer timer("agg_part_final", s);
    int form = DFF_PLAIN, tbk = tb;
    if (df.fx_q != 0.0 && only_set && !only_set->pad && only_set->regions > 0 && only_set->regions <= 512 && tb >= 7 && tb <= 13 &&
        (!df.has_side || (out != DF_TABLE && env_i64("VNM_DFX_LEAN_SIDE", 1))) && env_i64("VNM_DFX_LEAN", 1)) form = DFF_LEAN;
    else if (df.fx_q == 0.0 && lo64) {
        if (tb < 9 || tb > 12) return set_error("aggregate: no 64-bit compensation variant for this table size (internal error)");
        form = DFF_LO64;
    } else if (df.fx_q != 0.0) {
        if (tb < 7 || tb > 13) return set_error("aggregate: fixed-point entries with this table size (internal error)");
        form = DFF_FIXED;
    } else if (exact && (tb == 12 || tb == 13) && out != DF_TABLE) form = DFF_EXACT;
    else if (tb < 9 || tb > 12) tbk = 13;
    VNM_TRY((pick_int<7, 13>(tbk, [&](auto tbc) {
        return pick_out(out, [&](auto outc) { return launch_dense_final_as<decltype(tbc)::value, decltype(outc)::value>(form, df, only_set, s); });
    })));
    VNM_HIP(hipGetLastError());
    return 0;
}

int upload_segs(vnm_agg* h, int64_t tile, const VSeg** dev, int* nseg, int64_t* ntiles, PoolScope& pool, hipStream_t s) {
    const std::vector<vnm_agg::QBatch>& q = *h->segs_active;
    h->seg_host.resize(q.size());
    int64_t t = 0;
    for (size_t i = 0; i < q.size(); i++) {
        VSeg& g = h->seg_host[i];
        g.kp = (const uint64_t*)q[i].key.values + q[i].key.offset;
        g.vp = (const uint64_t*)q[i].col.values + q[i].col.offset;
        g.pp = h->pred_set ? (const double*)q[i].pred.values + q[i].pred.offset : nullptr;
        g.vvalid = nullptr; g.voff = 0;
        g.nrows = q[i].nrows;
        g.first_tile = t;
        t += (q[i].nrows + tile - 1) / tile;
    }
    VSeg* d = (VSeg*)pool.take(q.size() * sizeof(VSeg));
    if (!d) return 1;
    VNM_HIP(hipMemcpyAsync(d, h->seg_host.data(), q.size() * sizeof(VSeg), hipMemcpyHostToDevice, s));
    *dev = d; *nseg = (int)q.size(); *ntiles = t;
    return 0;
}

int complete_pending(vnm_agg* h, hipStream_t s, int out = DF_RUN, const DFinalArgs* cols = nullptr, int64_t* n_out = nullptr) {
    DensePending* pd = h->pending;
    if (!pd) return 0;
    if (out == DF_RUN && h->have_run) VNM_TRY(merge_run_into_table(h, s));
    DFinalArgs df = pd->df;
    PoolScope pool;
    uint64_t* rk = nullptr; uint64_t* ra = nullptr;
    if (out == DF_RUN) {
        rk = (uint64_t*)pool.take((size_t)pd->dstride * 8 * 2);
        ra = (uint64_t*)pool.take((size_t)pd->dstride * 8 * h->plan.n_words);
        if (!rk || !ra) return 1;
        df.dkey = rk; df.dacc = ra;
    } else if (out == DF_COLS) {
        df.n_out = cols->n_out;
        for (int c = 0; c < cols->n_out; c++) { df.out_kind[c] = cols->out_kind[c]; df.out_ptr[c] = cols->out_ptr[c]; df.key_field[c] = cols->key_field[c]; }
        df.pack_n = cols->pack_n;
        for (int j = 0; j < cols->pack_n; j++) { df.pack_shift[j] = cols->pack_shift[j]; df.pack_bits[j] = cols->pack_bits[j]; df.pack_lo[j] = cols->pack_lo[j]; }
        if (cols->has_side) { df.has_side = 1; df.side = cols->side; df.side_bloom = cols->side_bloom; df.side_bloom_mask = cols->side_bloom_mask; df.side_found = cols->side_found; }
    } else {
        if (!pd->table) pd->table = (DTabSlot*)pool_alloc(sizeof(DTabSlot) << df.map.bits);
        if (!pd->table) return 1;
        df.table = pd->table;
    }
    df.dstride = (out == DF_COLS && cols->dstride > 0) ? cols->dstride : pd->dstride;
    pool_free(pd->dsets);
    pd->dsets = (DSet*)pool_alloc(pd->sets.size() * sizeof(DSet));
    if (!pd->dsets) return 1;
    VNM_HIP(hipMemcpyAsync(pd->dsets, pd->sets.data(), pd->sets.size() * sizeof(DSet), hipMemcpyHostToDevice, s));
    df.sets = pd->dsets; df.nsets = (int)pd->sets.size();
    unsigned long long fl[5] = {0, 0, 0, 0, 0};
    uint64_t* psum = nullptr; float* plo = nullptr; uint32_t* pcnt = nullptr;
    if (pd->fsplits > 1 && df.has_side) return set_error("aggregate: side table with a split final pass (internal error)");
    if (pd->fsplits > 1) {
        const size_t cells = (size_t)pd->nfinal * pd->fsplits << pd->tb;
        psum = (uint64_t*)pool.take(cells * 8); plo = (float*)pool.take(cells * 4); pcnt = (uint32_t*)pool.take(cells * 4);
        if (!psum || !plo || !pcnt) return 1;
    }
    for (int attempt = 0; attempt < 2; attempt++) {
        VNM_HIP(hipMemsetAsync(df.flags, 0, 16, s));
        if (attempt == 0 && pd->fsplits > 1) {
            DFinalArgs ds = df;
            ds.splits = pd->fsplits; ds.part_sum = psum; ds.part_lo = plo; ds.part_cnt = pcnt;
            const int cus = device_info().num_cus;
            KernelTimer timer("agg_part_final", s);
            const int g3 = (int)std::min<int64_t>(pd->nfinal * pd->fsplits, (int64_t)cus * 8);
            if (pd->tb == 9) dpart_final_kernel<uint16_t, 9, true><<<g3, 512, 0, s>>>(ds);
            else if (pd->tb == 10) dpart_final_kernel<uint16_t, 10, true><<<g3, 512, 0, s>>>(ds);
            else if (pd->tb == 11) dpart_final_kernel<uint16_t, 11, true><<<g3, 512, 0, s>>>(ds);
            else if (pd->tb == 12) dpart_final_kernel<uint16_t, 12, true><<<g3, VNM_DF12_BLOCK, 0, s>>>(ds);
            else dpart_final_kernel<uint16_t, 13, true><<<g3, 1024, 0, s>>>(ds);
            if (out != DF_COLS) ds.n_out = 0;
            dpart_merge_kernel<<<(int)(pd->nfinal << (pd->tb - 9)), 512, 0, s>>>(ds, pd->tb);
            VNM_HIP(hipGetLastError());
        } else if (attempt == 1 && pd->tb == 13 && df.fx_q == 0.0) {
            df.sub_bits = 1;
            for (int sub = 0; sub < 2; sub++) { df.sub = sub; VNM_TRY(launch_dense_final(df, 12, out, true, s)); }
        } else {
            if (df.has_side) {
                VNM_HIP(hipMemsetAsync(df.side_found, 0, (size_t)df.side.cap + 2, s));
                VNM_HIP(hipMemsetAsync(df.flags + 4, 0, 8, s));
            }
            const int xmode = (int)env_i64("VNM_DF_EXACT", 1);
            const bool exact = attempt == 0 && df.w_sum >= 0 && df.w_lo >= 0 && !df.sub_bits && (xmode == 2 || (xmode == 1 && pd->exact_ok()));
            if (exact) route_note("dense:exact_adds", "2^%d-slot tables without compensation words: %lld rows, values below 2^%d with lowest bits >= 2^%d",
                                  pd->tb, (long long)pd->rows, (int)pd->x_exp - 1022, (int)(0xFFFFu - pd->x_inv) - 1075);
            VNM_TRY(launch_dense_final(df, pd->tb, out, attempt == 1, s, exact, pd->sets.size() == 1 ? &pd->sets[0] : nullptr));
            if (df.has_side) {
                KernelTimer timer("agg_side_append", s);
                dside_append_kernel<<<(int)std::min<int64_t>(((int64_t)df.side.cap + 2 + 255) / 256, (int64_t)device_info().num_cus * 8), 256, 0, s>>>(df, 0);
                dside_append_kernel<<<1, 256, 0, s>>>(df, 1);
                VNM_HIP(hipGetLastError());
            }
        }
        VNM_HIP(hipMemcpyAsync(fl, df.flags, 40, hipMemcpyDeviceToHost, s));
        VNM_HIP(hipStreamSynchronize(s));
        if (!fl[0]) break;
        if (out == DF_TABLE) return 2;
        if (attempt == 1) return set_error("aggregate: dense final pass failed (internal error)");
    }
    if (getenv("VNM_AGG_TRACE")) fprintf(stderr, "[agg] dense final (deferred, %zu batch%s): mode %d -> groups %llu\n", pd->sets.size(),
                                         pd->sets.size() == 1 ? "" : "es", out, fl[1]);
    if (n_out) *n_out = (int64_t)fl[1];
    if (out == DF_COLS && cols->null_pos) *cols->null_pos = df.has_side ? (int64_t)fl[4] : 0;
    if (out == DF_RUN) {
        pool.keep(rk); pool.keep(ra);
        h->run_key = rk; h->run_acc = ra; h->run_stride = pd->dstride; h->run_n = (int64_t)fl[1];
        h->run_dir = nullptr; h->run_nfin = 0;
        h->have_run = true;
        delete pd;
        h->pending = nullptr;
    }
    return 0;
}


struct DensePlan {
    bool generic, has_val;
    bool vn, vn_lists;
    bool fx_base;
    int tb, pbits, levels;
    int p1, p2, np1, np2;
    int64_t nfinal;
    int fsplits;
    bool count8;
    int c8_cb, c8_sub;
    bool fx;
    double fx_q;
    bool w32, w32_1;
    int grid1, split2;
    int64_t cap1, cap2;
    bool c16_1;
    int pmajor;
    int64_t spill_cap, nspill_cap, dstride;
    int rcap1, rcap2;
    bool ring_limit;
    int ring_pairs1, ring_pairs2;
};
constexpr int DENSE_REDO = 4;

int plan_dense_entries(const vnm_agg* h, const AggArgs& a, bool generic, const DGenArgs& g, bool vn_fold, bool null_lists, DensePlan* p) {
    p->generic = generic;
    p->has_val = generic ? g.has_val != 0 : true;
    if ((h->segs_active || h->kn_valid) && generic) return 2;
    if (h->kn_valid && h->segs_active) return 2;
    p->vn = p->has_val && a.cols[0].validity != nullptr && (generic || vn_fold);
    if (p->vn && ((!vn_fold && !null_lists) || a.has_expr)) return 2;
    if (vn_fold && (generic || !a.hot_pred_is_v)) return 2;
    p->vn_lists = p->vn && !vn_fold;
    p->fx_base = !generic && p->has_val && (!p->vn || vn_fold) && !a.has_expr && !(h->kn_valid && p->vn) && a.hot_comp && a.hot_w_sum >= 0 &&
                 env_i64("VNM_DENSE_DEFER", 1) && env_i64("VNM_DENSE_FX", 1) && a.cols[0].type == VNM_F64 && (env_i64("VNM_DENSE_RING", 3) & 3) == 3;
    return 0;
}

int sample_fixed_point(vnm_agg* h, const AggArgs& a, int64_t nrows, hipStream_t s) {
    h->fx_state = -1;
    PoolScope pool;
    unsigned long long* d = (unsigned long long*)pool.take(64);
    if (!d) return 1;
    unsigned long long got = 0;
    VNM_HIP(hipMemsetAsync(d, 0, 8, s));
    const int64_t srows = h->segs_active ? (*h->segs_active)[0].nrows : nrows;
    const int64_t m = std::min<int64_t>(srows, 1 << 16);
    fx_sample_kernel<<<(int)std::min<int64_t>((m + 255) / 256, 256), 256, 0, s>>>((const double*)a.cols[0].values + a.cols[0].offset, srows, m, d);
    VNM_HIP(hipGetLastError());
    VNM_HIP(hipMemcpyAsync(&got, d, 8, hipMemcpyDeviceToHost, s));
    VNM_HIP(hipStreamSynchronize(s));
    const uint32_t xinv = (uint32_t)got, xexp = (uint32_t)(got >> 32);
    if (xinv == 0 && xexp == 0) { h->fx_state = 1; h->fx_qe = -16; }
    else if (xexp < 2047) {
        const int L = (int)(0xFFFFu - xinv) - 1075, E = (int)xexp - 1022;
        const bool narrow = E - L <= 16 && env_i64("VNM_DENSE_FX_NARROW", 1) != 0;
        const int room = narrow ? 18 : 31;
        const int spare = room - (E - L);
        if (spare >= 0) {
            int qe = L - spare / 2;
            if (qe > 0) qe = 0;
            if (qe >= -1000 && E - qe <= room) { h->fx_state = 1; h->fx_qe = qe; h->fx_narrow = narrow; }
        }
    }
    if (getenv("VNM_AGG_TRACE")) fprintf(stderr, "[agg] fixed-point entries: sample says %s (qe %d)\n", h->fx_state == 1 ? "yes" : "no", h->fx_qe);
    return 0;
}

int plan_dense_geometry(const vnm_agg* h, const AggArgs& a, int64_t nrows, const DGenArgs& g, DensePlan* p) {
    const int cus = device_info().num_cus;
    const DenseMap& mp = h->dmap;
    const bool generic = p->generic, has_val = p->has_val;
    const bool fx_ok = p->fx_base && h->fx_state == 1;
    int tb = (int)env_i64("VNM_DENSE_TBITS", 12);
    tb = std::max(DP_TBITS_MIN, std::min(DP_TBITS_MAX, tb));
    while (tb > DP_TBITS_MIN && mp.bits - tb < 11) tb--;
    while (tb < DP_TBITS_MAX && mp.bits - tb > 18) tb++;
    const int one_level_bits = DP_TBITS_MAX + (has_val && env_i64("VNM_DENSE_ONE_LEVEL_512", 0) == 0 ? 8 : 9);
    if (mp.bits <= one_level_bits && env_i64("VNM_DENSE_ONE_LEVEL", 1)) tb = std::max(DP_TBITS_MIN, std::min(DP_TBITS_MAX, mp.bits - (int)env_i64("VNM_DENSE_ONE_P", 8)));
    if (mp.bits < 20) tb = (int)env_i64("VNM_DENSE_SMALL_TBITS", 11);
    if (mp.bits - tb < 5 && env_i64("VNM_DENSE_MIN_PARTS32", 1)) tb = std::max(9, mp.bits - 5);
    if (fx_ok && mp.bits >= 20 && mp.bits <= 22 && env_i64("VNM_DENSE_FX_ONE_LEVEL", 1)) tb = mp.bits - 9;
    const bool fx_small = fx_ok && mp.bits >= (int)env_i64("VNM_DENSE_FX_SMALL_MIN_BITS", 15) && mp.bits <= 19 && env_i64("VNM_DENSE_FX_SMALL", 1) != 0;
    if (fx_small) tb = std::max(7, mp.bits - 9);
    if (generic) {
        int tmax = DP_TBITS_MAX;
        while (tmax > 9 && ((size_t)dgen_slot_bytes(g) << tmax) > 64 * 1024) tmax--;
        if (mp.bits - tmax == 9 && tmax < DP_TBITS_MAX && ((size_t)dgen_slot_bytes(g) << (tmax + 1)) <= (size_t)env_i64("VNM_DGEN_BIG_LDS_KB", 128) * 1024) tmax++;
        if (((size_t)dgen_slot_bytes(g) << tmax) > 128 * 1024) return 2;
        if (tb > tmax) tb = tmax;
        if (mp.bits - tb > 18) return 2;
    }
    p->c8_cb = h->count_cb ? h->count_cb : ((h->hint == 0 || nrows <= 64 * h->hint) ? 8 : (nrows <= 16384 * h->hint ? 16 : 0));
    const int c8_tmax = p->c8_cb == 8 ? DC8_BITS : DC8_BITS - 1;
    p->count8 = generic && !has_val && g.n_lds == 0 && !p->vn && !h->count8_off && h->heavy_share == 0.0 && p->c8_cb != 0 && mp.bits >= DP_TBITS_MAX + 10 &&
                mp.bits <= c8_tmax + 9 + 1 && env_i64("VNM_DENSE_COUNT8", 1);
    p->c8_sub = p->count8 ? std::max(0, mp.bits - c8_tmax - 9) : 0;
    if (p->count8) tb = mp.bits - 9 - p->c8_sub;
    p->tb = tb;
    p->pbits = p->count8 ? 9 : mp.bits - tb;
    p->levels = p->pbits > 9 ? 2 : 1;
    const int pbits = p->pbits, levels = p->levels;
    p->nfinal = (int64_t)1 << pbits;
    int p1 = levels == 2 ? (int)env_i64("VNM_DENSE_P1", fx_ok ? (pbits + 1) / 2 : pbits / 2) : pbits;
    if (levels == 2) { if (p1 > 9) p1 = 9; if (pbits - p1 > 9) p1 = pbits - 9; }
    p->p1 = p1; p->p2 = pbits - p1;
    p->np1 = 1 << p1; p->np2 = levels == 2 ? 1 << p->p2 : 0;
    const int np1 = p->np1, np2 = p->np2;
    const int64_t tile1 = PT_TILE;
    const int grid1 = (int)std::min<int64_t>((int64_t)cus * env_i64("VNM_DENSE_GRID1_PER_CU", 2), (nrows + tile1 - 1) / tile1);
    int split2 = std::max(2, (grid1 + PT_MAX_REGIONS - 1) / PT_MAX_REGIONS);
    split2 = std::max(split2, std::min(grid1, (cus * 2 + np1 - 1) / np1));
    if (h->heavy_share > 0.0) split2 = std::min(grid1, split2 * (int)env_i64("VNM_DENSE_SKEW_SPLIT", 8));
    p->grid1 = grid1; p->split2 = split2;
    const int64_t tiles_per_wg = ((nrows + tile1 - 1) / tile1 + grid1 - 1) / grid1;
    const int64_t rows_per_wg = tiles_per_wg * tile1;
    int64_t cap1 = ((rows_per_wg / np1 + rows_per_wg / np1 / 5 + 512) + 15) & ~15LL;
    const bool odd_cap = env_i64("VNM_DENSE_ODD_CAP", 1) != 0;
    if (odd_cap && ((cap1 / 16) & 1) == 0) cap1 += 16;
    if (fx_ok && h->fx_narrow && levels == 1) { cap1 = (cap1 + 31) & ~31LL; if (((cap1 / 32) & 1) == 0) cap1 += 32; }
    p->cap1 = cap1;
    p->c16_1 = levels == 1 && !p->count8;
    int fsplits = 1;
    if (levels == 1 && !p->count8 && ((int64_t)1 << pbits) < (int64_t)cus * 2) {
        fsplits = (int)std::min<int64_t>(grid1, ((int64_t)cus * env_i64("VNM_DENSE_SPLIT_WGS", 4) + ((int64_t)1 << pbits) - 1) >> pbits);
        if (fsplits < 2) fsplits = 1;
    }
    if (fx_small && levels == 1) fsplits = 1;
    p->fsplits = fsplits;
    p->fx = fx_ok && fsplits == 1 && !p->count8 && tb >= (fx_small ? 7 : 11) && tb <= 13;
    p->fx_q = p->fx ? std::ldexp(1.0, h->fx_qe) : 0.0;
    p->w32 = p->fx && h->fx_narrow;
    p->w32_1 = p->w32 && levels == 1;
    if (levels == 2) {
        const int64_t per_pg = (int64_t)grid1 * rows_per_wg / np1 / split2;
        int64_t cap2 = ((per_pg / np2 + per_pg / np2 / 4 + 256) + 15) & ~15LL;
        if (odd_cap && ((cap2 / 16) & 1) == 0) cap2 += 16;
        if (p->w32) { cap2 = (cap2 + 31) & ~31LL; if (((cap2 / 32) & 1) == 0) cap2 += 32; }
        p->cap2 = cap2;
    }
    p->spill_cap = nrows / 2 + (1 << 20);
    p->nspill_cap = p->vn_lists ? nrows / 4 + (1 << 20) : 0;
    p->dstride = std::min<int64_t>(h->dense_span, nrows) + 2;
    p->pmajor = (int)env_i64("VNM_DENSE_PRODUCER_MAJOR", 0);
    const int use_ring = (int)env_i64("VNM_DENSE_RING", 3);
    p->ring_limit = env_i64("VNM_DENSE_RING_LIMIT", 1) != 0;
    p->rcap1 = p->w32_1 ? ring_cap_w32(np1) : ((use_ring & 1) && !a.has_expr ? ring_cap_for(np1, p->fx ? 8 : (has_val ? 8 : 0) + (p->c16_1 ? 2 : 4)) : 0);
    if (levels == 2) p->rcap2 = p->fx ? (p->w32 ? ring_cap_w32(np2) : ring_cap_for(np2, 8)) : ((use_ring & 2) ? ring_cap_for(np2, (has_val ? 8 : 0) + 2) : 0);
    p->ring_pairs1 = (int)env_i64("VNM_DENSE_RING_PAIRS", 4);
    if (p->fx && levels == 2 && getenv("VNM_DENSE_RING_PAIRS") == nullptr) p->ring_pairs1 = 2;
    p->ring_pairs2 = levels == 2 ? (int)env_i64("VNM_DENSE_RING_PAIRS2", p->fx && p->w32 ? 4 : 2) : 0;
    return 0;
}

struct DenseBuffers {
    PoolScope pool;
    unsigned long long* flags = nullptr;
    double* v1 = nullptr; void* c1 = nullptr; uint32_t* n1 = nullptr;
    double* v2 = nullptr; void* c2 = nullptr; uint32_t* n2 = nullptr;
    ulonglong2* spill = nullptr;
    uint64_t* nspill = nullptr;
    uint64_t* rk = nullptr; uint64_t* ra = nullptr;
    template <class T> void take(T*& p, size_t bytes) { p = (T*)pool.take(bytes); }
    void free_all() { while (pool.n > 0) pool.done(pool.blocks[pool.n - 1]); }
};

int dense_allocate(const DensePlan& p, DenseBuffers& b, hipStream_t s) {
    b.take(b.flags, 128);
    b.take(b.v1, p.has_val ? (size_t)p.np1 * p.grid1 * p.cap1 * (p.w32_1 ? 4 : 8) : 8);
    b.take(b.c1, p.fx ? 16 : (size_t)p.np1 * p.grid1 * p.cap1 * (p.c16_1 ? 2 : 4));
    b.take(b.n1, (size_t)p.np1 * p.grid1 * 4);
    b.take(b.spill, (size_t)p.spill_cap * 16);
    if (p.vn_lists) b.take(b.nspill, (size_t)p.nspill_cap * 8);
    if (!b.flags || !b.v1 || !b.c1 || !b.n1 || !b.spill || (p.vn_lists && !b.nspill)) return 1;
    VNM_HIP(hipMemsetAsync(b.flags, 0, 128, s));
    fill_u64_kernel<<<1, 1, 0, s>>>((uint64_t*)b.flags + 11, F64_NEG_ZERO, 1);
    VNM_HIP(hipGetLastError());
    return 0;
}

int fold_null_rows(const vnm_agg* h, const AggArgs& a, const unsigned long long* flags, hipStream_t s) {
    if (!h->kn_valid) return 0;
    const GTable& gt = h->g;
    const uint64_t slot = gt.cap + 1;
    dnull_fold_kernel<<<1, 64, 0, s>>>(flags + 8, gt.tag + slot,
                                       a.hot_w_rows >= 0 ? gt.acc + (uint64_t)a.hot_w_rows * gt.stride + slot : nullptr,
                                       a.hot_w_valid >= 0 ? gt.acc + (uint64_t)a.hot_w_valid * gt.stride + slot : nullptr,
                                       a.hot_w_sum >= 0 ? gt.acc + (uint64_t)a.hot_w_sum * gt.stride + slot : nullptr,
                                       a.hot_comp && a.hot_w_sum >= 0 ? (int64_t)gt.stride : 0);
    VNM_HIP(hipGetLastError());
    return 0;
}

int dense_scatter1_launch(vnm_agg* h, const DensePlan& p, DenseBuffers& b, DPartArgs& d1, hipStream_t s) {
    const bool pv = d1.has_pred && !d1.pred_is_v;
    if (!p.rcap1)
        return pick_bool(p.c16_1, [&](auto c16) {
            using CT = std::conditional_t<decltype(c16)::value, uint16_t, uint32_t>;
            if (p.vn) { dpart_scatter_kernel<true, CT, true, true><<<p.grid1, PT_BLOCK, 0, s>>>(d1); return 0; }
            return pick_bool(p.has_val, [&](auto hv) { dpart_scatter_kernel<true, CT, decltype(hv)::value><<<p.grid1, PT_BLOCK, 0, s>>>(d1); return 0; });
        });
    const bool plain_val = p.has_val && !p.vn;
    const RingLaunch r{p.grid1, p.rcap1, ring_sub_tile_pairs(p.ring_pairs1, pv, p.ring_limit, p.np1, p.rcap1, p.w32_1), p.ring_limit,
                       plain_val && h->segs_active != nullptr, plain_val && h->kn_valid != nullptr, s};
    if (r.seg && !r.kn && upload_segs(h, (int64_t)2 * r.pairs * 1024, &d1.segs, &d1.nseg, &d1.nsub, b.pool, s)) return 1;
    if (p.fx && p.vn)
        return pick_bool(p.w32_1, [&](auto w32) { return ring_scatter<true, uint32_t, true, false, true, true, decltype(w32)::value>(r, d1); });
    if (p.fx)
        return pick_bool(p.w32_1, [&](auto w32) {
            return pick_bool(pv, [&](auto pvc) { return ring_scatter<true, uint32_t, true, decltype(pvc)::value, false, true, decltype(w32)::value>(r, d1); });
        });
    return pick_bool(p.c16_1, [&](auto c16) {
        using CT = std::conditional_t<decltype(c16)::value, uint16_t, uint32_t>;
        return pick_bool(pv, [&](auto pvc) {
            if (p.vn) return ring_scatter<true, CT, true, decltype(pvc)::value, true>(r, d1);
            return pick_bool(p.has_val, [&](auto hv) { return ring_scatter<true, CT, decltype(hv)::value, decltype(pvc)::value, false>(r, d1); });
        });
    });
}

int dense_scatter1(vnm_agg* h, const AggArgs& a, int64_t nrows, const DensePlan& p, DenseBuffers& b, DPartArgs& d1, hipStream_t s) {
    d1.map = h->dmap;
    d1.kp = (const uint64_t*)a.keys[0].values + a.keys[0].offset;
    d1.vp = p.has_val ? (const double*)a.cols[0].values + a.cols[0].offset : nullptr;
    d1.has_expr = a.has_expr; d1.expr = a.expr;
    d1.pp = h->pred_set ? (const double*)a.pred.values + a.pred.offset : nullptr;
    d1.has_pred = h->pred_set; d1.pred_is_v = a.hot_pred_is_v; d1.op = a.p.op; d1.thr = a.p.dval;
    d1.nrows = nrows;
    d1.out_vals = b.v1; d1.out_codes = b.c1; d1.out_counts = b.n1; d1.out_cap = p.cap1;
    d1.nparts = p.np1; d1.out_bits = h->dmap.bits - p.p1;
    d1.producer_major = p.pmajor;
    d1.nt_store = (int)env_i64("VNM_DENSE_NT", p.levels == 2 && p.np2 >= 256 ? 1 : 0) & 1;
    d1.ready_list = (int)env_i64("VNM_DENSE_READY_LIST", 1) & 1;
    d1.flags = b.flags; d1.spill = b.spill; d1.spill_cap = p.spill_cap;
    d1.fx_q = p.fx_q; d1.fx_inv_q = p.fx ? std::ldexp(1.0, -h->fx_qe) : 0.0;
    d1.fx_lim = p.w32 ? (1LL << 18) - 1 : 2147483647LL;
    if (p.vn) { d1.vvalid = a.cols[0].validity; d1.voff = a.cols[0].offset; d1.nspill = b.nspill; d1.nspill_cap = p.nspill_cap; }
    if (h->kn_valid) {
        if (ensure_table(h, 1024, s, true)) return 1;
        uint64_t* scr = (uint64_t*)(b.flags + 8);
        d1.kvalid = h->kn_valid; d1.koff = h->kn_off;
        d1.nk_tag = scr;
        d1.nk_rows = a.hot_w_rows >= 0 ? scr + 1 : nullptr;
        d1.nk_valid = a.hot_w_valid >= 0 ? scr + 2 : nullptr;
        d1.nk_sum = a.hot_w_sum >= 0 ? scr + 3 : nullptr;
        d1.nk_lo_stride = a.hot_comp && a.hot_w_sum >= 0 ? 1 : 0;
    }
    {
        KernelTimer timer("agg_part_scatter1", s);
        VNM_TRY(dense_scatter1_launch(h, p, b, d1, s));
    }
    VNM_HIP(hipGetLastError());
    return 0;
}

int dense_scatter2(const vnm_agg* h, const DensePlan& p, DenseBuffers& b, const DPartArgs& d1, hipStream_t s) {
    b.take(b.v2, p.has_val ? (size_t)p.np1 * p.np2 * p.split2 * p.cap2 * (p.w32 ? 4 : 8) : 8);
    b.take(b.c2, p.fx ? 16 : (size_t)p.np1 * p.np2 * p.split2 * p.cap2 * 2);
    b.take(b.n2, (size_t)p.np1 * p.np2 * p.split2 * 4);
    if (!b.v2 || !b.c2 || !b.n2) return 1;
    DPartArgs d2{};
    d2.map = h->dmap;
    d2.in_vals = b.v1; d2.in_codes = (const uint32_t*)b.c1; d2.in_counts = b.n1; d2.in_cap = p.cap1;
    d2.in_regions = p.grid1; d2.in_split = p.split2; d2.in_bits = h->dmap.bits - p.p1;
    d2.in_pstride = p.pmajor ? 1 : p.grid1; d2.in_rstride = p.pmajor ? p.np1 : 1;
    d2.out_vals = b.v2; d2.out_codes = b.c2; d2.out_counts = b.n2; d2.out_cap = p.cap2;
    d2.nparts = p.np2; d2.out_bits = p.tb;
    d2.flags = b.flags; d2.spill = b.spill; d2.spill_cap = p.spill_cap;
    d2.nspill = b.nspill; d2.nspill_cap = p.nspill_cap;
    d2.nt_store = ((int)env_i64("VNM_DENSE_NT", 0) >> 1) & 1;
    d2.ready_list = ((int)env_i64("VNM_DENSE_READY_LIST", 1) >> 1) & 1;
    d2.fx_q = d1.fx_q; d2.fx_inv_q = d1.fx_inv_q; d2.fx_lim = d1.fx_lim;
    const int grid2 = p.np1 * p.split2;
    const RingLaunch r{grid2, p.rcap2, ring_sub_tile_pairs(p.ring_pairs2, false, p.ring_limit, p.np2, p.rcap2, p.w32), p.ring_limit, false, false, s};
    {
        KernelTimer timer("agg_part_scatter2", s);
        if (p.fx) VNM_TRY(pick_bool(p.w32, [&](auto w32) { return ring_scatter<false, uint32_t, true, false, false, true, decltype(w32)::value>(r, d2); }));
        else if (p.rcap2) VNM_TRY(pick_bool(p.has_val, [&](auto hv) { return ring_scatter<false, uint16_t, decltype(hv)::value, false, false>(r, d2); }));
        else VNM_TRY(pick_bool(p.has_val, [&](auto hv) { dpart_scatter_kernel<false, uint16_t, decltype(hv)::value><<<grid2, PT_BLOCK, 0, s>>>(d2); return 0; }));
    }
    VNM_HIP(hipGetLastError());
    return 0;
}

int dense_final_count8(vnm_agg* h, const DensePlan& p, const DenseBuffers& b, DGenArgs& g, hipStream_t s) {
    for (int cb = p.c8_cb;;) {
        const int tbc = std::min(p.tb, cb == 8 ? DC8_BITS : DC8_BITS - 1), subc = p.c8_sub + (p.tb - tbc);
        g.tbits = tbc;
        const size_t lds = ((size_t)1 << tbc) * (size_t)(cb / 8);
        {
            KernelTimer timer("agg_part_final", s);
            VNM_TRY(launch_resident(cb == 8 ? dcount8_final_kernel<8> : dcount8_final_kernel<16>, p.nfinal << subc, 1024, lds, 2, s, g, subc));
        }
        VNM_HIP(hipGetLastError());
        if (cb == 16) break;
        unsigned long long f6[6];
        VNM_HIP(hipMemcpyAsync(f6, b.flags, sizeof(f6), hipMemcpyDeviceToHost, s));
        VNM_HIP(hipStreamSynchronize(s));
        if (!(f6[0] && f6[5])) break;
        cb = 16;
        h->count_cb = 16;
        VNM_HIP(hipMemsetAsync(b.flags, 0, 16, s));
        VNM_HIP(hipMemsetAsync(b.flags + 5, 0, 8, s));
    }
    return 0;
}

int dense_final_generic(const DensePlan& p, DenseBuffers& b, DGenArgs& g, hipStream_t s) {
    const size_t slots = (size_t)1 << p.tb;
    const size_t lds = slots * dgen_slot_bytes(g);
    if (p.fsplits > 1) {
        const size_t work = (size_t)p.nfinal * p.fsplits;
        g.part_w = (uint64_t*)b.pool.take(std::max<size_t>(8, work * g.n_lds * slots * 8));
        g.part_cnt = (uint32_t*)b.pool.take(work * slots * 4);
        if (!g.part_w || !g.part_cnt) return 1;
        g.splits = p.fsplits;
    }
    KernelTimer timer("agg_part_final", s);
    VNM_TRY(pick_bool(p.has_val, [&](auto hv) {
        return pick_bool(p.fsplits > 1, [&](auto sp) {
            return launch_resident(dgen_final_kernel<decltype(hv)::value, decltype(sp)::value>, p.nfinal * (decltype(sp)::value ? p.fsplits : 1), 512, lds, 8, s, g);
        });
    }));
    if (p.fsplits > 1) dgen_merge_kernel<<<(int)(p.nfinal << (p.tb - 9)), 512, 0, s>>>(g);
    return 0;
}

int dense_final_split(const DensePlan& p, DenseBuffers& b, DFinalArgs& df, hipStream_t s) {
    const size_t cells = (size_t)p.nfinal * p.fsplits << p.tb;
    df.part_sum = (uint64_t*)b.pool.take(cells * 8); df.part_lo = (float*)b.pool.take(cells * 4); df.part_cnt = (uint32_t*)b.pool.take(cells * 4);
    if (!df.part_sum || !df.part_lo || !df.part_cnt) return 1;
    df.splits = p.fsplits;
    KernelTimer timer("agg_part_final", s);
    VNM_TRY((pick_int<9, 13>(p.tb >= 9 && p.tb <= 12 ? p.tb : 13, [&](auto tbc) {
        constexpr int TB = decltype(tbc)::value;
        return launch_resident(dpart_final_kernel<uint16_t, TB, true>, p.nfinal * p.fsplits, TB >= 13 ? 1024 : (TB == 12 ? VNM_DF12_BLOCK : 512), 0, 8, s, df);
    })));
    dpart_merge_kernel<<<(int)(p.nfinal << (p.tb - 9)), 512, 0, s>>>(df, p.tb);
    return 0;
}

int dense_defer_final(vnm_agg* h, const AggArgs& a, int64_t nrows, const DensePlan& p, DenseBuffers& b, const DSet& fin, DFinalArgs& df, hipStream_t s,
                      ulonglong2** spill_out, int64_t* n_spill_out) {
    const DenseMap& mp = h->dmap;
    unsigned long long fl0[8];
    VNM_HIP(hipMemcpyAsync(fl0, b.flags, 64, hipMemcpyDeviceToHost, s));
    VNM_HIP(hipStreamSynchronize(s));
    route_note(h->kn_valid ? "dense:nullable_key" : (h->segs_active ? "dense:stream_segments" : (p.vn ? "dense:nullable_value" : (p.levels == 1 && p.p1 == 5 && p.tb <= 10 ? "dense:32_partitions" :
               (p.fsplits > 1 ? "dense:split_final" : (p.levels == 2 ? "dense:two_levels" : "dense:one_level"))))),
               "2^%d codes, 2^%d-slot final tables, p1 %d p2 %d, final pass deferred%s: %s", mp.bits, p.tb, p.p1, p.p2, p.vn ? ", nullable value" : "", fl0[0] || (p.fx && fl0[7]) ? "scatter FAILED (the batch goes another way)" : "ok");
    if (getenv("VNM_AGG_TRACE"))
        fprintf(stderr, "[agg] dense: bits %d tb %d levels %d p1 %d p2 %d -> scatter fail %llu spilled %llu, final pass deferred (bound %lld)\n",
                mp.bits, p.tb, p.levels, p.p1, p.p2, fl0[0], fl0[2], (long long)p.dstride);
    if (p.fx && fl0[7]) {
        if (h->fx_narrow) {
            h->fx_narrow = false;
            h->fx_qe = std::max(h->fx_qe - 6, -1000);
            route_note("dense:fixed_point_misfit", "a value outside 2^%d * [-2^18, 2^18): the batch is redone with 64-bit entry words", h->fx_qe + 6);
            return DENSE_REDO;
        }
        h->fx_state = -1;
        route_note("dense:fixed_point_misfit", "a value outside 2^%d * [-2^31, 2^31): the batch is redone with float64 entries", h->fx_qe);
        return DENSE_REDO;
    }
    if (fl0[0]) return 2;
    if (p.fx) route_note("dense:fixed_point", "%s entry words, quantum 2^%d", p.w32 ? (p.levels == 1 ? "4-byte" : "8-byte, then 4-byte") : "8-byte", h->fx_qe);
    if (fold_null_rows(h, a, b.flags, s)) return 1;
    b.pool.done(b.rk); b.pool.done(b.ra);
    if (fl0[2]) { b.pool.keep(b.spill); *spill_out = b.spill; *n_spill_out = (int64_t)fl0[2]; }
    else { *spill_out = nullptr; *n_spill_out = 0; }
    if ((int64_t)fl0[2] > nrows / 16) h->dense_state = -1;
    DensePending* pd = h->pending;
    const int64_t pending_max_rows = std::min<int64_t>(env_i64("VNM_DENSE_PENDING_MAX_ROWS", 3LL << 29), (1LL << 32) - 1);
    if (pd && (pd->tb != p.tb || pd->levels != p.levels || pd->p1 != p.p1 || pd->fsplits != p.fsplits || pd->sets.size() >= DP_MAX_SETS ||
               pd->rows + nrows > pending_max_rows || pd->df.fx_q != p.fx_q || pd->df.fx_w32 != (p.w32 ? 1 : 0) || memcmp(&pd->df.map, &mp, sizeof(DenseMap)) != 0)) {
        VNM_TRY(complete_pending(h, s));
        pd = nullptr;
    }
    if (!pd) {
        pd = new DensePending();
        df.dkey = nullptr; df.dacc = nullptr;
        pd->df = df; pd->tb = p.tb; pd->levels = p.levels; pd->p1 = p.p1; pd->fsplits = p.fsplits; pd->nfinal = p.nfinal; pd->dstride = 0;
        b.pool.keep(b.flags); pd->blocks.push_back(b.flags);
        h->pending = pd;
    }
    pd->dstride = std::min<int64_t>(h->dense_span, pd->dstride + nrows) + 2;
    pd->rows += nrows;
    if (p.rcap1 && p.has_val && !a.has_expr && !p.fx) { pd->x_inv = std::max(pd->x_inv, (uint32_t)fl0[6]); pd->x_exp = std::max(pd->x_exp, (uint32_t)(fl0[6] >> 32)); }
    else pd->x_known = false;
    pd->sets.push_back(fin);
    void* const held[3] = {p.levels == 2 ? (void*)b.v2 : (void*)b.v1, p.levels == 2 ? b.c2 : b.c1, p.levels == 2 ? (void*)b.n2 : (void*)b.n1};
    for (void* blk : held) { b.pool.keep(blk); pd->blocks.push_back(blk); }
    return 0;
}

int dense_hand_over(vnm_agg* h, const AggArgs& a, int64_t nrows, const DensePlan& p, DenseBuffers& b, hipStream_t s, ulonglong2** spill_out, int64_t* n_spill_out,
                    uint64_t** nspill_out, int64_t* n_nspill_out) {
    VNM_HIP(hipGetLastError());
    unsigned long long fl[4];
    VNM_HIP(hipMemcpyAsync(fl, b.flags, 32, hipMemcpyDeviceToHost, s));
    VNM_HIP(hipStreamSynchronize(s));
    if (!fl[0]) {
        if (fold_null_rows(h, a, b.flags, s)) return 1;
        VNM_HIP(hipStreamSynchronize(s));
    }
    route_note(p.count8 ? "dense:count_bytes" : p.generic ? (p.fsplits > 1 ? "dense:generic_split_final" : "dense:generic") : (p.vn ? "dense:nullable_value" : (p.fsplits > 1 ? "dense:split_final" : "dense:run")),
               "2^%d codes, 2^%d-slot final tables, levels %d, p1 %d p2 %d, %d final splits: %s", h->dmap.bits, p.tb, p.levels, p.p1, p.p2, p.fsplits, fl[0] ? "FAILED (the batch goes another way)" : "ok");
    if (getenv("VNM_AGG_TRACE"))
        fprintf(stderr, "[agg] dense%s%s: bits %d tb %d levels %d p1 %d p2 %d splits %d -> fail %llu groups %llu spilled %llu + %llu NULL-value rows (dstride %lld)\n",
                p.generic ? " generic" : "", p.vn ? " nullable" : "", h->dmap.bits, p.tb, p.levels, p.p1, p.p2, p.fsplits, fl[0], fl[1], fl[2], fl[3], (long long)p.dstride);
    if (fl[0]) {
        if (!p.count8) return 2;
        h->count8_off = true;
        return DENSE_REDO;
    }
    if (fl[2]) { b.pool.keep(b.spill); *spill_out = b.spill; *n_spill_out = (int64_t)fl[2]; }
    else { *spill_out = nullptr; *n_spill_out = 0; }
    if (p.vn && fl[3]) { b.pool.keep(b.nspill); *nspill_out = b.nspill; *n_nspill_out = (int64_t)fl[3]; }
    if ((int64_t)(fl[2] + fl[3]) > nrows / 16) h->dense_state = -1;
    b.pool.keep(b.rk); b.pool.keep(b.ra);
    h->run_key = b.rk; h->run_acc = b.ra; h->run_stride = p.dstride; h->run_n = (int64_t)fl[1];
    h->run_dir = nullptr; h->run_nfin = 0;
    h->have_run = true;
    return 0;
}

int dense_partitioned_aggregate(vnm_agg* h, const AggArgs& a, int64_t nrows, hipStream_t s, ulonglong2** spill_out, int64_t* n_spill_out,
                                bool generic = false, uint64_t** nspill_out = nullptr, int64_t* n_nspill_out = nullptr, bool vn_fold = false) {
    DGenArgs g{};
    if (generic && !dgen_program(h, a, &g)) return 2;
    DensePlan p{};
    VNM_TRY(plan_dense_entries(h, a, generic, g, vn_fold, nspill_out != nullptr, &p));
    if (nspill_out) { *nspill_out = nullptr; *n_nspill_out = 0; }
    if (p.fx_base && h->fx_state == 0) VNM_TRY(sample_fixed_point(h, a, nrows, s));
    VNM_TRY(plan_dense_geometry(h, a, nrows, g, &p));
    DenseBuffers b;
    auto redo = [&]() { b.free_all(); return dense_partitioned_aggregate(h, a, nrows, s, spill_out, n_spill_out, generic, nspill_out, n_nspill_out, vn_fold); };
    VNM_TRY(dense_allocate(p, b, s));
    if (p.fx && (!p.rcap1 || (p.levels == 2 && !p.rcap2))) { h->fx_state = -1; return redo(); }
    if ((h->segs_active || h->kn_valid) && (!p.rcap1 || p.vn)) return 2;
    DPartArgs d1{};
    VNM_TRY(dense_scatter1(h, a, nrows, p, b, d1, s));
    if (p.levels == 2) VNM_TRY(dense_scatter2(h, p, b, d1, s));
    DSet fin{b.v1, b.c1, b.n1, p.cap1, p.grid1, 1, p.grid1, 0};
    if (p.levels == 2) fin = DSet{b.v2, b.c2, b.n2, p.cap2, p.split2, 1, p.split2, 0};
    else if (p.pmajor) { fin.pstride = 1; fin.rstride = p.np1; }
    fin.pad = fin.cap < 2048 ? 1 : 0;
    b.take(b.rk, (size_t)p.dstride * 8 * 2);
    b.take(b.ra, (size_t)p.dstride * 8 * h->plan.n_words);
    if (!b.rk || !b.ra) return 1;
    DFinalArgs df{};
    df.map = h->dmap;
    df.vals = fin.vals; df.codes = fin.codes; df.counts = fin.counts; df.cap = fin.cap; df.regions = fin.regions; df.nfinal = p.nfinal;
    df.pstride = fin.pstride; df.rstride = fin.rstride;
    df.w_rows = a.hot_w_rows; df.w_valid = a.hot_w_valid; df.w_sum = a.hot_w_sum;
    df.w_lo = a.hot_comp && a.hot_w_sum >= 0 ? a.hot_w_sum + 1 : -1;
    df.dkey = b.rk; df.dacc = b.ra; df.dstride = p.dstride; df.flags = b.flags;
    df.fx_q = p.fx_q; df.fx_w32 = p.w32 ? 1 : 0;
    const bool own_run = generic || !env_i64("VNM_DENSE_DEFER", 1);
    if (own_run && h->pending) {
        int rc = complete_pending(h, s);
        if (!rc) rc = merge_run_into_table(h, s);
        if (rc) return 1;
    }
    if (generic) {
        g.map = h->dmap; g.tbits = p.tb;
        g.pstride = fin.pstride; g.rstride = fin.rstride;
        g.vals = p.count8 ? nullptr : fin.vals; g.codes = fin.codes; g.counts = fin.counts; g.cap = fin.cap; g.regions = fin.regions; g.nfinal = p.nfinal;
        g.dkey = b.rk; g.dacc = b.ra; g.dstride = p.dstride; g.flags = b.flags;
    }
    if (p.count8) VNM_TRY(dense_final_count8(h, p, b, g, s));
    else if (generic) VNM_TRY(dense_final_generic(p, b, g, s));
    else if (p.fsplits > 1 && own_run) VNM_TRY(dense_final_split(p, b, df, s));
    else if (env_i64("VNM_DENSE_DEFER", 1)) {
        const int rc = dense_defer_final(h, a, nrows, p, b, fin, df, s, spill_out, n_spill_out);
        return rc == DENSE_REDO ? redo() : rc;
    } else VNM_TRY(launch_dense_final(df, p.tb, DF_RUN, false, s));
    const int rc = dense_hand_over(h, a, nrows, p, b, s, spill_out, n_spill_out, nspill_out, n_nspill_out);
    return rc == DENSE_REDO ? redo() : rc;
}


int dense_two_aggregate(vnm_agg* h, const AggArgs& a, int64_t nrows, hipStream_t s) {
    const int cus = device_info().num_cus;
    const DenseMap& mp = h->dmap;
    int tb = 11;
    if (mp.bits - tb > 15) tb = 12;
    const int pbits = mp.bits - tb;
    if (pbits > 15 || pbits < 10 || a.has_expr) return 2;
    const int p2 = std::min(8, (pbits + 1) / 2), p1 = pbits - p2;
    if (p1 > 7 || p1 < 5) return 2;
    const int np1 = 1 << p1, np2 = 1 << p2;
    const int64_t tile1 = PT_TILE;
    const int grid1 = (int)std::min<int64_t>((int64_t)cus * 2, (nrows + tile1 - 1) / tile1);
    int split2 = std::max(2, (grid1 + PT_MAX_REGIONS - 1) / PT_MAX_REGIONS);
    split2 = std::max(split2, std::min(grid1, (cus * 2 + np1 - 1) / np1));
    const int64_t tiles_per_wg = ((nrows + tile1 - 1) / tile1 + grid1 - 1) / grid1;
    const int64_t rows_per_wg = tiles_per_wg * tile1;
    int64_t cap1 = ((rows_per_wg / np1 + rows_per_wg / np1 / 5 + 512) + 15) & ~15LL;
    if (((cap1 / 16) & 1) == 0) cap1 += 16;
    const int64_t per_pg = (int64_t)grid1 * rows_per_wg / np1 / split2;
    int64_t cap2 = ((per_pg / np2 + per_pg / np2 / 4 + 256) + 15) & ~15LL;
    if (((cap2 / 16) & 1) == 0) cap2 += 16;
    const int64_t nfinal = (int64_t)1 << pbits;
    const int64_t dstride = std::min<int64_t>(h->dense_span, nrows) + 2;
    PoolScope pool;
    unsigned long long* flags = (unsigned long long*)pool.take(64);
    double* v1 = (double*)pool.take((size_t)np1 * grid1 * cap1 * 8);
    double* w1 = (double*)pool.take((size_t)np1 * grid1 * cap1 * 8);
    uint32_t* c1 = (uint32_t*)pool.take((size_t)np1 * grid1 * cap1 * 4);
    uint32_t* n1 = (uint32_t*)pool.take((size_t)np1 * grid1 * 4);
    double* v2 = (double*)pool.take((size_t)np1 * np2 * split2 * cap2 * 8);
    double* w2 = (double*)pool.take((size_t)np1 * np2 * split2 * cap2 * 8);
    uint16_t* c2 = (uint16_t*)pool.take((size_t)np1 * np2 * split2 * cap2 * 2);
    uint32_t* n2 = (uint32_t*)pool.take((size_t)np1 * np2 * split2 * 4);
    uint64_t* rk = (uint64_t*)pool.take((size_t)dstride * 8 * 2);
    uint64_t* ra = (uint64_t*)pool.take((size_t)dstride * 8 * h->plan.n_words);
    if (!flags || !v1 || !w1 || !c1 || !n1 || !v2 || !w2 || !c2 || !n2 || !rk || !ra) return 1;
    VNM_HIP(hipMemsetAsync(flags, 0, 64, s));
// ... 70 lines not shown
```

Before: 148.4 billion rows/s.

## Use 32-bit windowed fixed-point words out of the first of two dense levels

With two scatter levels, the first level now packs each entry into a 32-bit word: a coarser fixed-point quantum plus a value window. The window base is planned from a sampled value min/max that the sample kernel now also returns. The second level reads these 4-byte words with vectorized uint4 loads and adds the base back. This halves the intermediate partition traffic between the levels, which previously used 8-byte words. A value outside the window sets a new flag bit, disables the mode and redoes the batch with 8-byte words, so a poor sample costs a redo.

```diff
diff --git a/vinum_amd/csrc/vnm_agg.hip b/vinum_amd/csrc/vnm_agg.hip
--- a/vinum_amd/csrc/vnm_agg.hip
+++ b/vinum_amd/csrc/vnm_agg.hip
@@ -373,6 +373,9 @@
     bool pack_null_seen = false;
     bool pring_off = false;
     bool fx_narrow = false;
+    int fx_L = 0, fx_E = 0;
+    double fx_vmin = 0.0, fx_vmax = 0.0;
+    bool fx_narrow1_off = false;
     int fxn_state = 0, fxn_qe[3] = {0, 0, 0};
     bool null_inputs_seen = false;
     bool count8_off = false;
diff --git a/vinum_amd/csrc/vnm_agg_dense.inc b/vinum_amd/csrc/vnm_agg_dense.inc
--- a/vinum_amd/csrc/vnm_agg_dense.inc
+++ b/vinum_amd/csrc/vnm_agg_dense.inc
@@ -65,6 +65,7 @@
     int64_t nspill_cap;
     double fx_q, fx_inv_q;
     int64_t fx_lim;
+    int fx_wbits, fx_wbase, fx_wuns, fx_sh, fx_in_base;
 };
 constexpr uint32_t DP_NULL32 = 0x80000000u;
 __device__ __forceinline__ bool fx_encode(double v, double inv_q, int64_t* m, int64_t lim = 2147483647LL) {
@@ -337,11 +338,13 @@
 typedef double dr_v2 __attribute__((ext_vector_type(2)));
 typedef uint32_t dr_u2 __attribute__((ext_vector_type(2)));
 template <bool FROM_ROWS, typename CT, bool HAS_VAL, int DR_BLOCK, int DR_PAIRS, bool PV = false, bool VN = false, int MAXR = 0, bool SEG = false, bool KN = false,
-          bool V2 = false, bool FX = false, bool W32 = false>
+          bool V2 = false, bool FX = false, bool W32 = false, bool IN32 = false, bool WIN = false>
 __global__ __launch_bounds__(DR_BLOCK) void dring_scatter_kernel(DPartArgs a, int ring_cap) {
     extern __shared__ uint64_t dr_lds[];
     static_assert(!FX || (HAS_VAL && !V2), "fixed-point entries: one value (VN: only where the filter drops the NULL rows, vn_fold)");
     static_assert(!W32 || FX, "32-bit entry words are fixed-point words");
+    static_assert(!IN32 || (W32 && !FROM_ROWS), "32-bit input words: the second of two levels of 32-bit fixed-point words");
+    static_assert(!WIN || (W32 && FROM_ROWS), "window words: 32-bit words out of the first of two levels");
     constexpr int FB = W32 ? 32 : DR_FB, EPL = FB / 8;
     constexpr int NE = 2 * DR_PAIRS;
     const int np = a.nparts;
@@ -385,7 +388,7 @@
         uint32_t slot = head[p] + r;
         if (slot >= (uint32_t)ring_cap) slot -= ring_cap;
         if (W32) {
-            ((uint32_t*)rv)[(size_t)p * ring_cap + slot] = ((uint32_t)(int32_t)fx_of(v) << a.out_bits) | (c & remmask);
+            ((uint32_t*)rv)[(size_t)p * ring_cap + slot] = ((uint32_t)((int32_t)fx_of(v) - (WIN ? a.fx_wbase : 0)) << a.out_bits) | (c & remmask);
             return true;
         }
         if (FX) {
@@ -399,7 +402,12 @@
     };
     auto fx_rem = [&](size_t li) -> uint32_t { return W32 ? ((const uint32_t*)rv)[li] & remmask : (uint32_t)(((const uint64_t*)rv)[li] & (uint64_t)remmask); };
     auto fx_val = [&](size_t li) -> double {
-        return W32 ? (double)((int32_t)((const uint32_t*)rv)[li] >> a.out_bits) * a.fx_q : (double)((int64_t)((const uint64_t*)rv)[li] >> a.out_bits) * a.fx_q;
+        if (W32) {
+            const uint32_t w = ((const uint32_t*)rv)[li];
+            if (WIN) return (double)((a.fx_wuns ? (int32_t)(w >> a.out_bits) : (int32_t)w >> a.out_bits) + a.fx_wbase) * a.fx_q;
+            return (double)((int32_t)w >> a.out_bits) * a.fx_q;
+        }
+        return (double)((int64_t)((const uint64_t*)rv)[li] >> a.out_bits) * a.fx_q;
     };
     auto flush = [&](bool drain) {
         const int j = tid & 7;
@@ -534,7 +542,18 @@
     uint32_t nk_cnt = 0;
     constexpr bool XT = FROM_ROWS && HAS_VAL && !V2 && !FX;
     uint32_t xinv = 0, xexp = 0;
-    bool fx_bad = false;
+    uint32_t fx_bad = 0;
+    auto fx_entry = [&](double val, double* out) -> bool {
+        int64_t m;
+        if (!fx_encode(val, a.fx_inv_q, &m, a.fx_lim)) { fx_bad |= 1u; return false; }
+        if (WIN) {
+            const int64_t m1 = m >> a.fx_sh;
+            if ((m1 << a.fx_sh) != m || (uint64_t)(m1 - (int64_t)a.fx_wbase) >> a.fx_wbits) { fx_bad |= 2u; return false; }
+            m = m1;
+        }
+        *out = fx_bits(m);
+        return true;
+    };
     if (FROM_ROWS && !SEG) {
         const int64_t sub = (int64_t)NE * DR_BLOCK;
         const int64_t nsub = (a.nrows + sub - 1) / sub;
@@ -600,7 +619,7 @@
                 }
                 c[e] = (((uint32_t)d * a.map.mul) & a.map.mask) | (VN && isnull ? DP_NULL32 : 0u);
                 v[e] = VN && isnull ? 0.0 : val;
-                if (FX) { int64_t m; if (!fx_encode(val, a.fx_inv_q, &m, a.fx_lim)) { fx_bad = true; continue; } v[e] = fx_bits(m); }
+                if (FX && !fx_entry(val, &v[e])) continue;
                 if (V2) w2[V2 ? e : 0] = val2;
                 if (XT) exact_track(v[e], xinv, xexp);
                 okmask |= 1u << e;
@@ -666,7 +685,7 @@
                 if (d > (uint64_t)a.map.mask) { dense_spill(a, key, val, isnull); continue; }
                 c[e] = (((uint32_t)d * a.map.mul) & a.map.mask) | (VN && isnull ? DP_NULL32 : 0u);
                 v[e] = VN && isnull ? 0.0 : val;
-                if (FX) { int64_t m; if (!fx_encode(val, a.fx_inv_q, &m, a.fx_lim)) { fx_bad = true; continue; } v[e] = fx_bits(m); }
+                if (FX && !fx_entry(val, &v[e])) continue;
                 if (XT) exact_track(v[e], xinv, xexp);
                 okmask |= 1u << e;
             }
@@ -683,61 +702,84 @@
         const int first = g * per_max;
         const int per = first + per_max <= a.in_regions ? per_max : (a.in_regions > first ? a.in_regions - first : 0);
         const int64_t region0 = (int64_t)pin * a.in_pstride + (int64_t)first * a.in_rstride;
+        constexpr int IU = IN32 ? (DR_PAIRS >= 2 ? 4 : 2) : 2, NU = NE / IU;
         if (tid == 0) {
             uint32_t run = 0;
-            for (int rj = 0; rj < per; rj++) { rstart[rj] = run; run += (a.in_counts[region0 + rj * a.in_rstride] + 1) / 2; }
+            for (int rj = 0; rj < per; rj++) { rstart[rj] = run; run += (a.in_counts[region0 + rj * a.in_rstride] + IU - 1) / IU; }
             rstart[per] = run;
         }
         __syncthreads();
         const uint32_t total_in = rstart[per];
-        double2 ev[DR_PAIRS], ev2[V2 ? DR_PAIRS : 1];
-        uint2 ec[DR_PAIRS];
+        double2 ev[IN32 ? 1 : DR_PAIRS], ev2[V2 ? DR_PAIRS : 1];
+        uint2 ec[IN32 ? 1 : DR_PAIRS];
+        uint32_t ew[IN32 ? NE : 1];
         uint32_t okm = 0;
         int reg = 0;
         auto load_pairs = [&](uint32_t t0) {
             okm = 0;
 #pragma unroll
-            for (int u = 0; u < DR_PAIRS; u++) {
+            for (int u = 0; u < NU; u++) {
                 const uint32_t v = t0 + (uint32_t)u * DR_BLOCK + tid;
                 if (v < total_in) {
                     int lo = reg;
                     while (rstart[lo + 1] <= v) lo++;
                     reg = lo;
-                    const uint32_t e0 = 2u * (v - rstart[lo]);
+                    const uint32_t e0 = (uint32_t)IU * (v - rstart[lo]);
                     const int64_t rg = region0 + lo * a.in_rstride;
                     const int64_t at = rg * a.in_cap + e0;
-                    if (HAS_VAL) ev[u] = *(const double2*)(a.in_vals + at);
+                    if (IN32) {
+                        const uint32_t* src = (const uint32_t*)a.in_vals + at;
+                        if (IU == 4) { const uint4 x = *(const uint4*)src; ew[IN32 ? 4 * u : 0] = x.x; ew[IN32 ? 4 * u + 1 : 0] = x.y; ew[IN32 ? 4 * u + 2 : 0] = x.z; ew[IN32 ? 4 * u + 3 : 0] = x.w; }
+                        else { const uint2 x = *(const uint2*)src; ew[IN32 ? 2 * u : 0] = x.x; ew[IN32 ? 2 * u + 1 : 0] = x.y; }
+                        const uint32_t left = a.in_counts[rg] - e0;
+                        okm |= (left >= (uint32_t)IU ? (1u << IU) - 1u : (1u << left) - 1u) << (IU * u);
+                        continue;
+                    }
+                    if (HAS_VAL) ev[IN32 ? 0 : u] = *(const double2*)(a.in_vals + at);
                     if (V2) ev2[V2 ? u : 0] = *(const double2*)(a.in_vals2 + at);
-                    if (!FX) ec[u] = *(const uint2*)(a.in_codes + at);
+                    if (!FX) ec[IN32 ? 0 : u] = *(const uint2*)(a.in_codes + at);
                     okm |= (e0 + 1 < a.in_counts[rg] ? 3u : 1u) << (2 * u);
                 }
             }
         };
         load_pairs(0);
-        for (uint32_t t0 = 0; t0 < total_in; t0 += DR_PAIRS * DR_BLOCK) {
+        for (uint32_t t0 = 0; t0 < total_in; t0 += NU * DR_BLOCK) {
             uint32_t c[NE]; double v[NE]; double w2[V2 ? NE : 1];
-#pragma unroll
-            for (int u = 0; u < DR_PAIRS; u++) {
-                if (FX) {
-                    const uint64_t w0 = (uint64_t)__double_as_longlong(ev[u].x), w1 = (uint64_t)__double_as_longlong(ev[u].y);
-                    const uint64_t inmask = ((uint64_t)1 << a.in_bits) - 1;
-                    c[2 * u] = (uint32_t)(w0 & inmask); c[2 * u + 1] = (uint32_t)(w1 & inmask);
-                    v[2 * u] = fx_bits((int64_t)w0 >> a.in_bits); v[2 * u + 1] = fx_bits((int64_t)w1 >> a.in_bits);
-                    continue;
-                }
-                c[2 * u] = ec[u].x; c[2 * u + 1] = ec[u].y;
-                v[2 * u] = HAS_VAL ? ev[u].x : 0.0; v[2 * u + 1] = HAS_VAL ? ev[u].y : 0.0;
-                if (V2) { w2[V2 ? 2 * u : 0] = ev2[V2 ? u : 0].x; w2[V2 ? 2 * u + 1 : 0] = ev2[V2 ? u : 0].y; }
+            if (IN32) {
+                const uint32_t inmask = (1u << a.in_bits) - 1u;
+#pragma unroll
+                for (int e = 0; e < NE; e++) {
+                    const uint32_t w = ew[IN32 ? e : 0];
+                    c[e] = w & inmask;
+                    v[e] = fx_bits((int64_t)((int32_t)(w >> a.in_bits) + a.fx_in_base));
+                }
+            } else {
+#pragma unroll
+                for (int u = 0; u < DR_PAIRS; u++) {
+                    if (FX) {
+                        const uint64_t w0 = (uint64_t)__double_as_longlong(ev[IN32 ? 0 : u].x), w1 = (uint64_t)__double_as_longlong(ev[IN32 ? 0 : u].y);
+                        const uint64_t inmask = ((uint64_t)1 << a.in_bits) - 1;
+                        c[2 * u] = (uint32_t)(w0 & inmask); c[2 * u + 1] = (uint32_t)(w1 & inmask);
+                        v[2 * u] = fx_bits((int64_t)w0 >> a.in_bits); v[2 * u + 1] = fx_bits((int64_t)w1 >> a.in_bits);
+                        continue;
+                    }
+                    c[2 * u] = ec[IN32 ? 0 : u].x; c[2 * u + 1] = ec[IN32 ? 0 : u].y;
+                    v[2 * u] = HAS_VAL ? ev[IN32 ? 0 : u].x : 0.0; v[2 * u + 1] = HAS_VAL ? ev[IN32 ? 0 : u].y : 0.0;
+                    if (V2) { w2[V2 ? 2 * u : 0] = ev2[V2 ? u : 0].x; w2[V2 ? 2 * u + 1 : 0] = ev2[V2 ? u : 0].y; }
+                }
             }
             const uint32_t okmask = okm;
-            load_pairs(t0 + DR_PAIRS * DR_BLOCK);
+            load_pairs(t0 + NU * DR_BLOCK);
             rounds(c, v, w2, okmask);
         }
     }
     flush(true);
     __syncthreads();
     if (tid < np) a.out_counts[out_base + (int64_t)tid * out_stride] = cursor[tid];
-    if (FX && FROM_ROWS) { if (__syncthreads_or(fx_bad ? 1 : 0) && tid == 0) __hip_atomic_store(&a.flags[7], 1ULL, __ATOMIC_RELAXED, __HIP_MEMORY_SCOPE_AGENT); }
+    if (FX && FROM_ROWS) {
+        const int bad0 = __syncthreads_or((int)(fx_bad & 1u)), bad1 = WIN ? __syncthreads_or((int)(fx_bad & 2u)) : 0;
+        if ((bad0 || bad1) && tid == 0) __hip_atomic_fetch_or(&a.flags[7], (bad0 ? 1ULL : 0ULL) | (bad1 ? 2ULL : 0ULL), __ATOMIC_RELAXED, __HIP_MEMORY_SCOPE_AGENT);
+    }
     if (XT) {
         if (tid < 2) s_spill[tid] = 0;
         __syncthreads();
@@ -2127,17 +2169,38 @@
     }
 }
 
-__global__ __launch_bounds__(256) void fx_sample_kernel(const double* vals, int64_t nrows, int64_t m, unsigned long long* out) {
+__host__ __device__ __forceinline__ unsigned long long f64_ordered(double v) {
+    unsigned long long b;
+    memcpy(&b, &v, 8);
+    return (b >> 63) ? ~b : b | 0x8000000000000000ULL;
+}
+__host__ __device__ __forceinline__ double f64_of_ordered(unsigned long long u) {
+    const unsigned long long b = (u >> 63) ? u & 0x7FFFFFFFFFFFFFFFULL : ~u;
+    double v;
+    memcpy(&v, &b, 8);
+    return v;
+}
+__global__ __launch_bounds__(256) void fx_sample_kernel(const double* vals, int64_t nrows, int64_t m, unsigned long long* out, unsigned long long* mm = nullptr) {
     __shared__ uint32_t sx[2];
-    if (threadIdx.x < 2) sx[threadIdx.x] = 0;
+    __shared__ unsigned long long smm[2];
+    if (threadIdx.x < 2) { sx[threadIdx.x] = 0; smm[threadIdx.x] = 0; }
     __syncthreads();
     const int64_t stride = (int64_t)gridDim.x * blockDim.x;
     uint32_t xinv = 0, xexp = 0;
-    for (int64_t i = (int64_t)blockIdx.x * blockDim.x + threadIdx.x; i < m; i += stride) exact_track(vals[(int64_t)(((__int128)i * nrows) / m)], xinv, xexp);
+    unsigned long long nmin = 0, vmax = 0;
+    for (int64_t i = (int64_t)blockIdx.x * blockDim.x + threadIdx.x; i < m; i += stride) {
+        const double v = vals[(int64_t)(((__int128)i * nrows) / m)];
+        exact_track(v, xinv, xexp);
+        const unsigned long long u = f64_ordered(v);
+        nmin = ~u > nmin ? ~u : nmin;
+        vmax = u > vmax ? u : vmax;
+    }
     if (xinv) atomicMax(&sx[0], xinv);
     if (xexp) atomicMax(&sx[1], xexp);
+    if (mm && vmax) { atomicMax(&smm[0], nmin); atomicMax(&smm[1], vmax); }
     __syncthreads();
     if (threadIdx.x < 2 && sx[threadIdx.x]) atomicMax((uint32_t*)out + threadIdx.x, sx[threadIdx.x]);
+    if (mm && threadIdx.x < 2 && smm[threadIdx.x]) atomicMax(&mm[threadIdx.x], smm[threadIdx.x]);
 }
 
 __global__ __launch_bounds__(256) void dense_sample_range_kernel(const uint64_t* keys, int64_t nrows, int64_t m, uint64_t sign,
diff --git a/vinum_amd/csrc/vnm_agg_routes.inc b/vinum_amd/csrc/vnm_agg_routes.inc
--- a/vinum_amd/csrc/vnm_agg_routes.inc
+++ b/vinum_amd/csrc/vnm_agg_routes.inc
@@ -61,16 +61,16 @@
     return cap >= 64 ? cap : 0;
 }
 
-template <bool FR, typename CT, bool HV, int PR, bool PV, bool VN, int MAXR, bool SEG, bool KN, bool V2, bool FX, bool W32>
+template <bool FR, typename CT, bool HV, int PR, bool PV, bool VN, int MAXR, bool SEG, bool KN, bool V2, bool FX, bool W32, bool IN32 = false, bool WIN = false>
 int launch_ring(int grid, const DPartArgs& d, int cap, hipStream_t s) {
     constexpr size_t esize = FX ? (W32 ? 4 : 8) : (HV ? (V2 ? 16 : 8) : 0) + sizeof(CT);
     const size_t lds = (((size_t)d.nparts * cap * esize) + 15) & ~(size_t)15;
-    return launch_dyn(dring_scatter_kernel<FR, CT, HV, 1024, PR, PV, VN, MAXR, SEG, KN, V2, FX, W32>, grid, 1024, lds, s, d, cap);
-}
-template <bool FR, typename CT, bool HV, bool PV, bool VN, bool FX, bool W32, int PR>
+    return launch_dyn(dring_scatter_kernel<FR, CT, HV, 1024, PR, PV, VN, MAXR, SEG, KN, V2, FX, W32, IN32, WIN>, grid, 1024, lds, s, d, cap);
+}
+template <bool FR, typename CT, bool HV, bool PV, bool VN, bool FX, bool W32, int PR, bool IN32 = false, bool WIN = false>
 int ring_scatter_pairs(const RingLaunch& r, const DPartArgs& d) {
     auto go = [&](auto lim, auto seg, auto kn) {
-        return launch_ring<FR, CT, HV, PR, PV, VN, decltype(lim)::value ? 2 : 0, decltype(seg)::value, decltype(kn)::value, false, FX, W32>(r.grid, d, r.cap, r.s);
+        return launch_ring<FR, CT, HV, PR, PV, VN, decltype(lim)::value ? 2 : 0, decltype(seg)::value, decltype(kn)::value, false, FX, W32, IN32, WIN>(r.grid, d, r.cap, r.s);
     };
     return pick_bool(r.limit && ring_one_round(PR, d.nparts, r.cap, W32), [&](auto lim) {
         if constexpr (FR && HV && !VN) {
@@ -80,13 +80,13 @@
         return go(lim, std::false_type{}, std::false_type{});
     });
 }
-template <bool FR, typename CT, bool HV, bool PV, bool VN, bool FX = false, bool W32 = false>
+template <bool FR, typename CT, bool HV, bool PV, bool VN, bool FX = false, bool W32 = false, bool IN32 = false, bool WIN = false>
 int ring_scatter(const RingLaunch& r, const DPartArgs& d) {
     if constexpr (!PV) {
-        if (r.pairs == 4) return ring_scatter_pairs<FR, CT, HV, PV, VN, FX, W32, 4>(r, d);
-    }
-    if (r.pairs >= 2) return ring_scatter_pairs<FR, CT, HV, PV, VN, FX, W32, 2>(r, d);
-    return ring_scatter_pairs<FR, CT, HV, PV, VN, FX, W32, 1>(r, d);
+        if (r.pairs == 4) return ring_scatter_pairs<FR, CT, HV, PV, VN, FX, W32, 4, IN32, WIN>(r, d);
+    }
+    if (r.pairs >= 2) return ring_scatter_pairs<FR, CT, HV, PV, VN, FX, W32, 2, IN32, WIN>(r, d);
+    return ring_scatter_pairs<FR, CT, HV, PV, VN, FX, W32, 1, IN32, WIN>(r, d);
 }
 
 
@@ -724,6 +724,9 @@
     bool fx;
     double fx_q;
     bool w32, w32_1;
+    bool narrow1;
+    int fx_qe;
+    int fx_wbits, fx_wbase;
     int grid1, split2;
     int64_t cap1, cap2;
     bool c16_1;
@@ -754,18 +757,21 @@
     PoolScope pool;
     unsigned long long* d = (unsigned long long*)pool.take(64);
     if (!d) return 1;
-    unsigned long long got = 0;
-    VNM_HIP(hipMemsetAsync(d, 0, 8, s));
+    unsigned long long got3[3] = {0, 0, 0};
+    VNM_HIP(hipMemsetAsync(d, 0, 24, s));
     const int64_t srows = h->segs_active ? (*h->segs_active)[0].nrows : nrows;
     const int64_t m = std::min<int64_t>(srows, 1 << 16);
-    fx_sample_kernel<<<(int)std::min<int64_t>((m + 255) / 256, 256), 256, 0, s>>>((const double*)a.cols[0].values + a.cols[0].offset, srows, m, d);
+    fx_sample_kernel<<<(int)std::min<int64_t>((m + 255) / 256, 256), 256, 0, s>>>((const double*)a.cols[0].values + a.cols[0].offset, srows, m, d, d + 1);
     VNM_HIP(hipGetLastError());
-    VNM_HIP(hipMemcpyAsync(&got, d, 8, hipMemcpyDeviceToHost, s));
+    VNM_HIP(hipMemcpyAsync(got3, d, 24, hipMemcpyDeviceToHost, s));
     VNM_HIP(hipStreamSynchronize(s));
+    const unsigned long long got = got3[0];
     const uint32_t xinv = (uint32_t)got, xexp = (uint32_t)(got >> 32);
-    if (xinv == 0 && xexp == 0) { h->fx_state = 1; h->fx_qe = -16; }
-    else if (xexp < 2047) {
-        const int L = (int)(0xFFFFu - xinv) - 1075, E = (int)xexp - 1022;
+    const bool zeros = xinv == 0 && xexp == 0;
+    if (zeros || xexp < 2047) {
+        const int L = zeros ? 0 : (int)(0xFFFFu - xinv) - 1075, E = zeros ? 0 : (int)xexp - 1022;
+        h->fx_L = L; h->fx_E = E;
+        h->fx_vmin = zeros ? 0.0 : f64_of_ordered(~got3[1]); h->fx_vmax = zeros ? 0.0 : f64_of_ordered(got3[2]);
         const bool narrow = E - L <= 16 && env_i64("VNM_DENSE_FX_NARROW", 1) != 0;
         const int room = narrow ? 18 : 31;
         const int spare = room - (E - L);
@@ -775,8 +781,26 @@
             if (qe >= -1000 && E - qe <= room) { h->fx_state = 1; h->fx_qe = qe; h->fx_narrow = narrow; }
         }
     }
-    if (getenv("VNM_AGG_TRACE")) fprintf(stderr, "[agg] fixed-point entries: sample says %s (qe %d)\n", h->fx_state == 1 ? "yes" : "no", h->fx_qe);
-    return 0;
+    if (getenv("VNM_AGG_TRACE")) fprintf(stderr, "[agg] fixed-point entries: sample says %s (qe %d, values %g .. %g)\n", h->fx_state == 1 ? "yes" : "no", h->fx_qe, h->fx_vmin, h->fx_vmax);
+    return 0;
+}
+
+bool plan_narrow_first_level(const vnm_agg* h, int bits, int pbits, bool p1_given, int* p1, int* qe_out, int* wbits, int* wbase) {
+    if (!h->fx_narrow || h->fx_narrow1_off || env_i64("VNM_DENSE_FX_NARROW", 1) == 2) return false;
+    for (int pc = *p1; pc <= 9 && (pc == *p1 || (!p1_given && pbits - pc >= 5)); pc++) {
+        const int v1 = 32 - (bits - pc);
+        if (v1 < 1 || v1 > 24) continue;
+        const int room = std::min(18, v1);
+        int qe = h->fx_E - h->fx_L <= room ? h->fx_L - (room - (h->fx_E - h->fx_L)) / 2 : h->fx_L;
+        qe = std::max(std::min(qe, 0), h->fx_qe);
+        const int64_t mn = (int64_t)std::ldexp(h->fx_vmin, -qe), mx = (int64_t)std::ldexp(h->fx_vmax, -qe);
+        const int64_t w = (int64_t)1 << v1;
+        if (mx - mn >= w) continue;
+        *p1 = pc; *qe_out = qe; *wbits = v1;
+        *wbase = mn >= 0 && mx < w ? 0 : (mx <= 0 && mn > -w ? (int)(1 - w) : (int)(mn - (w - 1 - (mx - mn)) / 2));
+        return true;
+    }
+    return false;
 }
 
 int plan_dense_geometry(const vnm_agg* h, const AggArgs& a, int64_t nrows, const DGenArgs& g, DensePlan* p) {
@@ -816,6 +840,8 @@
     p->nfinal = (int64_t)1 << pbits;
     int p1 = levels == 2 ? (int)env_i64("VNM_DENSE_P1", fx_ok ? (pbits + 1) / 2 : pbits / 2) : pbits;
     if (levels == 2) { if (p1 > 9) p1 = 9; if (pbits - p1 > 9) p1 = pbits - 9; }
+    p->fx_qe = h->fx_qe; p->fx_wbits = 0; p->fx_wbase = 0;
+    p->narrow1 = fx_ok && levels == 2 && tb >= 11 && tb <= 13 && plan_narrow_first_level(h, mp.bits, pbits, getenv("VNM_DENSE_P1") != nullptr, &p1, &p->fx_qe, &p->fx_wbits, &p->fx_wbase);
     p->p1 = p1; p->p2 = pbits - p1;
     p->np1 = 1 << p1; p->np2 = levels == 2 ? 1 << p->p2 : 0;
     const int np1 = p->np1, np2 = p->np2;
@@ -830,7 +856,7 @@
     int64_t cap1 = ((rows_per_wg / np1 + rows_per_wg / np1 / 5 + 512) + 15) & ~15LL;
     const bool odd_cap = env_i64("VNM_DENSE_ODD_CAP", 1) != 0;
     if (odd_cap && ((cap1 / 16) & 1) == 0) cap1 += 16;
-    if (fx_ok && h->fx_narrow && levels == 1) { cap1 = (cap1 + 31) & ~31LL; if (((cap1 / 32) & 1) == 0) cap1 += 32; }
+    if (fx_ok && h->fx_narrow && (levels == 1 || p->narrow1)) { cap1 = (cap1 + 31) & ~31LL; if (((cap1 / 32) & 1) == 0) cap1 += 32; }
     p->cap1 = cap1;
     p->c16_1 = levels == 1 && !p->count8;
     int fsplits = 1;
@@ -841,9 +867,10 @@
     if (fx_small && levels == 1) fsplits = 1;
     p->fsplits = fsplits;
     p->fx = fx_ok && fsplits == 1 && !p->count8 && tb >= (fx_small ? 7 : 11) && tb <= 13;
-    p->fx_q = p->fx ? std::ldexp(1.0, h->fx_qe) : 0.0;
+    if (!p->fx) p->narrow1 = false;
+    p->fx_q = p->fx ? std::ldexp(1.0, p->fx_qe) : 0.0;
     p->w32 = p->fx && h->fx_narrow;
-    p->w32_1 = p->w32 && levels == 1;
+    p->w32_1 = p->w32 && (levels == 1 || p->narrow1);
     if (levels == 2) {
         const int64_t per_pg = (int64_t)grid1 * rows_per_wg / np1 / split2;
         int64_t cap2 = ((per_pg / np2 + per_pg / np2 / 4 + 256) + 15) & ~15LL;
@@ -916,6 +943,10 @@
     const RingLaunch r{p.grid1, p.rcap1, ring_sub_tile_pairs(p.ring_pairs1, pv, p.ring_limit, p.np1, p.rcap1, p.w32_1), p.ring_limit,
                        plain_val && h->segs_active != nullptr, plain_val && h->kn_valid != nullptr, s};
     if (r.seg && !r.kn && upload_segs(h, (int64_t)2 * r.pairs * 1024, &d1.segs, &d1.nseg, &d1.nsub, b.pool, s)) return 1;
+    if (p.fx && p.narrow1) {
+        if (p.vn) return ring_scatter<true, uint32_t, true, false, true, true, true, false, true>(r, d1);
+        return pick_bool(pv, [&](auto pvc) { return ring_scatter<true, uint32_t, true, decltype(pvc)::value, false, true, true, false, true>(r, d1); });
+    }
     if (p.fx && p.vn)
         return pick_bool(p.w32_1, [&](auto w32) { return ring_scatter<true, uint32_t, true, false, true, true, decltype(w32)::value>(r, d1); });
     if (p.fx)
@@ -947,6 +978,7 @@
     d1.flags = b.flags; d1.spill = b.spill; d1.spill_cap = p.spill_cap;
     d1.fx_q = p.fx_q; d1.fx_inv_q = p.fx ? std::ldexp(1.0, -h->fx_qe) : 0.0;
     d1.fx_lim = p.w32 ? (1LL << 18) - 1 : 2147483647LL;
+    if (p.narrow1) { d1.fx_wbits = p.fx_wbits; d1.fx_wbase = p.fx_wbase; d1.fx_wuns = 1; d1.fx_sh = p.fx_qe - h->fx_qe; }
     if (p.vn) { d1.vvalid = a.cols[0].validity; d1.voff = a.cols[0].offset; d1.nspill = b.nspill; d1.nspill_cap = p.nspill_cap; }
     if (h->kn_valid) {
         if (ensure_table(h, 1024, s, true)) return 1;
@@ -983,11 +1015,13 @@
     d2.nt_store = ((int)env_i64("VNM_DENSE_NT", 0) >> 1) & 1;
     d2.ready_list = ((int)env_i64("VNM_DENSE_READY_LIST", 1) >> 1) & 1;
     d2.fx_q = d1.fx_q; d2.fx_inv_q = d1.fx_inv_q; d2.fx_lim = d1.fx_lim;
+    d2.fx_in_base = d1.fx_wbase;
     const int grid2 = p.np1 * p.split2;
     const RingLaunch r{grid2, p.rcap2, ring_sub_tile_pairs(p.ring_pairs2, false, p.ring_limit, p.np2, p.rcap2, p.w32), p.ring_limit, false, false, s};
     {
         KernelTimer timer("agg_part_scatter2", s);
-        if (p.fx) VNM_TRY(pick_bool(p.w32, [&](auto w32) { return ring_scatter<false, uint32_t, true, false, false, true, decltype(w32)::value>(r, d2); }));
+        if (p.fx && p.narrow1) VNM_TRY((ring_scatter<false, uint32_t, true, false, false, true, true, true>(r, d2)));
+        else if (p.fx) VNM_TRY(pick_bool(p.w32, [&](auto w32) { return ring_scatter<false, uint32_t, true, false, false, true, decltype(w32)::value>(r, d2); }));
         else if (p.rcap2) VNM_TRY(pick_bool(p.has_val, [&](auto hv) { return ring_scatter<false, uint16_t, decltype(hv)::value, false, false>(r, d2); }));
         else VNM_TRY(pick_bool(p.has_val, [&](auto hv) { dpart_scatter_kernel<false, uint16_t, decltype(hv)::value><<<grid2, PT_BLOCK, 0, s>>>(d2); return 0; }));
     }
@@ -1064,6 +1098,11 @@
     if (getenv("VNM_AGG_TRACE"))
         fprintf(stderr, "[agg] dense: bits %d tb %d levels %d p1 %d p2 %d -> scatter fail %llu spilled %llu, final pass deferred (bound %lld)\n",
                 mp.bits, p.tb, p.levels, p.p1, p.p2, fl0[0], fl0[2], (long long)p.dstride);
+    if (p.fx && fl0[7] == 2) {
+        h->fx_narrow1_off = true;
+        route_note("dense:fixed_point_misfit", "a value outside the first level's window, 2^%d * [%d, %d + 2^%d): the batch is redone with 8-byte words out of that level", p.fx_qe, p.fx_wbase, p.fx_wbase, p.fx_wbits);
+        return DENSE_REDO;
+    }
     if (p.fx && fl0[7]) {
         if (h->fx_narrow) {
             h->fx_narrow = false;
@@ -1076,7 +1115,9 @@
         return DENSE_REDO;
     }
     if (fl0[0]) return 2;
-    if (p.fx) route_note("dense:fixed_point", "%s entry words, quantum 2^%d", p.w32 ? (p.levels == 1 ? "4-byte" : "8-byte, then 4-byte") : "8-byte", h->fx_qe);
+    if (p.fx) route_note("dense:fixed_point", "%s entry words, quantum 2^%d", p.w32 ? (p.levels == 1 ? "4-byte" : (p.narrow1 ? "4-byte, then 4-byte" : "8-byte, then 4-byte")) : "8-byte", p.fx_qe);
+    if (p.w32 && !p.narrow1) route_note("dense:fixed_point_narrow_last_level", "32-bit words out of the last of %d level(s) only", p.levels);
+    if (p.narrow1) route_note("dense:fixed_point_narrow_levels", "32-bit words out of both levels: p1 %d, a window of %d bits from %d quanta of 2^%d", p.p1, p.fx_wbits, p.fx_wbase, p.fx_qe);
     if (fold_null_rows(h, a, b.flags, s)) return 1;
     b.pool.done(b.rk); b.pool.done(b.ra);
     if (fl0[2]) { b.pool.keep(b.spill); *spill_out = b.spill; *n_spill_out = (int64_t)fl0[2]; }
```

Measured after the change: 158.1 billion rows/s (median of 6 runs). 6.6% higher.
